# r9y9/gantts

Measured on NVIDIA H100. Metric: gan_step_frames_per_sec, higher is better.
Workload: dtype f32 (GEMMs: bf16x3 split on wgmma, fp32 accumulate)

## Files before the change

### gantts_b200/csrc/gan_step.cu

```cuda
#include <nvtx3/nvToolsExt.h>

#include "common.cuh"

namespace gantts {

struct NvtxRange {
  explicit NvtxRange(const char* name) { nvtxRangePushA(name); }
  ~NvtxRange() { nvtxRangePop(); }
};

enum ScalarSlot {
  S_REAL = 0,
  S_FAKE = 3,
  S_ADV = 6,
  S_MGE = 9,
  S_MSE = 11,
  S_DSUMSQ = 13,
  S_GSUMSQ = 14,
  S_INV_T = 15,
  S_ADV_SCALE = 16,
  S_MGE_SCALE = 17,
  S_MSE_SCALE = 18,
  S_COUNT = 32
};

__global__ void gather_cols_list_kernel(const float* __restrict__ in, int64_t in_rs, float* __restrict__ out,
                                        int64_t out_rs, ColList cols, int64_t rows) {
  __shared__ int sc[GANTTS_MAX_COLS];
  for (int i = threadIdx.x; i < cols.n; i += blockDim.x) sc[i] = cols.c[i];
  __syncthreads();
  const int lane = threadIdx.x & 31;
  const int64_t warp = ((int64_t)blockIdx.x * blockDim.x + threadIdx.x) >> 5;
  const int64_t nwarps = ((int64_t)gridDim.x * blockDim.x) >> 5;
  for (int64_t r = warp; r < rows; r += nwarps)
    for (int j = lane; j < cols.n; j += 32) out[r * out_rs + j] = in[r * in_rs + sc[j]];
}

__global__ void gather_planes_kernel(const float* __restrict__ a, int64_t a_rs, ColList ca, int64_t rows_a,
                                     const float* __restrict__ b, int64_t b_rs, ColList cb, int64_t rows_b,
                                     __nv_bfloat16* __restrict__ hi, __nv_bfloat16* __restrict__ lo, int64_t pitch) {
  pdl_entry();
  __shared__ int sa[GANTTS_MAX_COLS], sb[GANTTS_MAX_COLS];
  for (int i = threadIdx.x; i < ca.n; i += blockDim.x) sa[i] = ca.c[i];
  for (int i = threadIdx.x; i < cb.n; i += blockDim.x) sb[i] = cb.c[i];
  __syncthreads();
  const int lane = threadIdx.x & 31;
  const int64_t warp = ((int64_t)blockIdx.x * blockDim.x + threadIdx.x) >> 5;
  const int64_t nwarps = ((int64_t)gridDim.x * blockDim.x) >> 5;
  for (int64_t r = warp; r < rows_a + rows_b; r += nwarps) {
    const bool first = r < rows_a;
    const float* src = first ? a + r * a_rs : b + (r - rows_a) * b_rs;
    const int* sc = first ? sa : sb;
    const int n = first ? ca.n : cb.n;
    uint32_t* hr = reinterpret_cast<uint32_t*>(hi + r * pitch);
    uint32_t* lr = reinterpret_cast<uint32_t*>(lo + r * pitch);
    for (int c = 2 * lane; c < n; c += 64) {
      const float v0 = src[sc[c]], v1 = (c + 1 < n) ? src[sc[c + 1]] : 0.f;
      const uint32_t hp = pack_bf16x2(v0, v1);
      hr[c >> 1] = hp;
      lr[c >> 1] = pack_bf16x2(v0 - __uint_as_float(hp << 16), v1 - __uint_as_float(hp & 0xffff0000u));
    }
  }
}

__global__ void scatter_cols_list_add_kernel(const float* __restrict__ go, int64_t go_rs, float* __restrict__ gi,
                                             int64_t gi_rs, ColList cols, int64_t rows) {
  __shared__ int sc[GANTTS_MAX_COLS];
  for (int i = threadIdx.x; i < cols.n; i += blockDim.x) sc[i] = cols.c[i];
  __syncthreads();
  const int lane = threadIdx.x & 31;
  const int64_t warp = ((int64_t)blockIdx.x * blockDim.x + threadIdx.x) >> 5;
  const int64_t nwarps = ((int64_t)gridDim.x * blockDim.x) >> 5;
  for (int64_t r = warp; r < rows; r += nwarps)
    for (int j = lane; j < cols.n; j += 32) gi[r * gi_rs + sc[j]] += go[r * go_rs + j];
}

__global__ void set_scales_kernel(float* scal, float inv_frames, float adv_w, float mge_w, float mse_w,
                                  int zero_norms, const int64_t* __restrict__ lengths, int B, int T) {
  pdl_entry();
  if (threadIdx.x == 0) {
    if (zero_norms) scal[S_DSUMSQ] = scal[S_GSUMSQ] = 0.f;
    if (!(inv_frames > 0.f)) {
      int64_t n = 0;
      for (int b = 0; b < B; ++b) {
        const int64_t l = lengths[b];
        n += l < 0 ? 0 : (l > T ? T : l);
      }
      inv_frames = n > 0 ? 1.f / (float)n : 0.f;
    }
    scal[S_INV_T] = inv_frames;
    scal[S_ADV_SCALE] = adv_w * inv_frames;
    scal[S_MGE_SCALE] = mge_w * inv_frames;
    scal[S_MSE_SCALE] = mse_w * inv_frames;
  }
}

__global__ void __launch_bounds__(RED_THREADS)
spoof_count_kernel(const float* __restrict__ Dv, const int64_t* __restrict__ lengths, int B, int T, float* __restrict__ count) {
  pdl_entry();
  __shared__ float sm[32];
  float v[1] = {0.f};
  const int64_t rows = (int64_t)B * T;
  for (int64_t r = threadIdx.x; r < rows; r += RED_THREADS) {
    const int64_t t = r % T;
    if (t < lengths[r / T] && Dv[r] > 0.5f) v[0] += 1.f;
  }
  block_sum<1>(v, sm);
  if (threadIdx.x == 0) count[0] = v[0];
}

enum RedSlot { R_REAL = 0, R_FAKE = 1, R_ADV = 2, R_MGE = 3, R_MSE = 4, R_COUNT = 5 };

struct RedCounts {
  int n[R_COUNT];
};

__global__ void __launch_bounds__(RED_THREADS)
finalize_losses_kernel(const float* scal, float* losses, const RedWs* red, RedCounts cnt, float adv_w, float mge_w,
                       float mse_w, int has_d) {
  pdl_entry();
  __shared__ float sm[RED_NV * 32];
  __shared__ float tot[R_COUNT][RED_NV];
  for (int sl = 0; sl < R_COUNT; ++sl) {
    float v[RED_NV] = {0.f, 0.f, 0.f, 0.f};
    for (int i = threadIdx.x; i < cnt.n[sl]; i += RED_THREADS) {
#pragma unroll
      for (int k = 0; k < RED_NV; ++k) v[k] += red[sl].partial[i][k];
    }
    block_sum<RED_NV>(v, sm);
    if (threadIdx.x == 0) {
#pragma unroll
      for (int k = 0; k < RED_NV; ++k) tot[sl][k] = v[k];
    }
    __syncthreads();
  }
  if (threadIdx.x != 0) return;
  const float invT = scal[S_INV_T];
  const float real = has_d ? tot[R_REAL][0] * invT : 0.f, fake = has_d ? tot[R_FAKE][0] * invT : 0.f;
  const float adv = (has_d && adv_w > 0.f) ? tot[R_ADV][0] * invT : 0.f;
  const float mge = tot[R_MGE][0] * invT, mse = tot[R_MSE][0] * invT;
  losses[0] = real + fake;
  losses[1] = fake;
  losses[2] = real;
  losses[3] = mse;
  losses[4] = mge;
  losses[5] = adv;
  losses[6] = (mse_w * mse + mge_w * mge) + adv_w * adv;
  losses[7] = has_d ? tot[R_REAL][1] : 0.f;
  losses[8] = has_d ? tot[R_FAKE][1] : 0.f;
  losses[9] = tot[R_MGE][1];
  losses[10] = has_d ? sqrtf(scal[S_DSUMSQ]) : 0.f;
  losses[11] = sqrtf(scal[S_GSUMSQ]);
}

static inline int blocks_1d(int64_t work, int per_block) {
  int64_t b = (work + per_block - 1) / per_block;
  if (b < 1) b = 1;
  if (b > 132 * 8) b = 132 * 8;
  return (int)b;
}

static_assert(GANTTS_MAX_STEP_TENSORS == OPT_MAX_TENSORS, "one model's tensor table is one TensorList of the clip kernels");
static_assert(2 + 2 * GANTTS_MAX_LAYERS <= GANTTS_MAX_STEP_TENSORS && 2 * GANTTS_MAX_SRU_LAYERS + 2 <= GANTTS_MAX_STEP_TENSORS &&
                  2 + 8 * GANTTS_MAX_LSTM_LAYERS + 2 <= GANTTS_MAX_STEP_TENSORS,
              "every generator the step accepts fits one tensor table");

struct Bound {
  float* p;
  float* g;
};
enum { WEIGHT = 0, BIAS = 1 };
enum { W_IH = 0, W_HH = 1, B_IH = 2, B_HH = 3 };

struct ParamList {
  int n;
  float* p[GANTTS_MAX_STEP_TENSORS];
  float* g[GANTTS_MAX_STEP_TENSORS];
  float* s[GANTTS_MAX_STEP_TENSORS];
  float* s2[GANTTS_MAX_STEP_TENSORS];
  int64_t sizes[GANTTS_MAX_STEP_TENSORS];
  int64_t total;
  Bound gate[2];
  Bound sru[GANTTS_MAX_SRU_LAYERS][2];
  Bound lstm[GANTTS_MAX_LSTM_LAYERS][2][4];
  float* gW[GANTTS_MAX_LAYERS];
  float* gb[GANTTS_MAX_LAYERS];
};

static inline size_t al256(size_t v) { return (v + 255) / 256 * 256; }

struct Arena {
  char* cur;
  char* take(size_t bytes) {
    char* p = cur;
    cur += al256(bytes);
    return p;
  }
  float* f32(size_t n) { return reinterpret_cast<float*>(take(n * sizeof(float))); }
};

struct HighwayWs {
  float* tx;
  float* gx;
  char* w;
  char* dz;
  float* partial;
};

struct SruWs {
  char* in[GANTTS_MAX_SRU_LAYERS];
  float* u[GANTTS_MAX_SRU_LAYERS];
  float* c[GANTTS_MAX_SRU_LAYERS];
  float* h[GANTTS_MAX_SRU_LAYERS];
  char* w[GANTTS_MAX_SRU_LAYERS];
  float* partial[GANTTS_MAX_SRU_LAYERS];
  char* du;
  float* dx;
  float* dxp;
  float* bpart;
};

struct LstmWs {
  char* in[GANTTS_MAX_LSTM_LAYERS];
  char* w[GANTTS_MAX_LSTM_LAYERS];
  float* bias[GANTTS_MAX_LSTM_LAYERS];
  float* h[GANTTS_MAX_LSTM_LAYERS];
  float* gates[GANTTS_MAX_LSTM_LAYERS];
  float* cells[GANTTS_MAX_LSTM_LAYERS];
  float* xproj;
  float* out;
  float* dh;
  char* dg;
  char* hp;
  float* part[2][2];
  unsigned int* bar;
  int64_t* lengths;
};

struct StepLayout {
  float* scal;
  float* mask;
  float* d_in;
  float* d_out;
  float* g_dout;
  float* g_din;
  float* g_static;
  float* g_yhat;
  float* g_grads;
  float* d_grads;
  char* g_tape;
  size_t g_tape_bytes;
  char* d_tape;
  size_t d_tape_bytes;
  char* mlp_ws;
  size_t mlp_ws_bytes;
  RedWs* red;
  float* opt_partial;
  HighwayWs hw;
  SruWs sru;
  LstmWs lstm;
  LstmWs d_lstm;
  size_t total;
};

static inline int sru_ncols(const gantts_sru_stack_t& s) { return s.hidden * (s.bidirectional ? 2 : 1); }
static inline int sru_nin(const gantts_sru_stack_t& s, int l) { return l == 0 ? s.in_dim : sru_ncols(s); }
static inline int sru_k(const gantts_sru_stack_t& s, int l) { return sru_nin(s, l) != sru_ncols(s) ? 4 : 3; }
static inline int lstm_ndir(const gantts_lstm_stack_t& s) { return s.bidirectional ? 2 : 1; }
static inline int lstm_nin(const gantts_lstm_stack_t& s, int l) { return l == 0 ? s.in_dim : lstm_ndir(s) * s.hidden; }

static inline int gen_in_width(const gantts_gan_step_t* c) {
  return c->sru.num_layers > 0 ? c->sru.in_dim : (c->lstm.num_layers > 0 ? c->lstm.in_dim : c->g.dims[0]);
}

static inline int d_in_width(const gantts_gan_step_t* c) {
  return c->d_lstm.num_layers > 0 ? c->d_lstm.in_dim : c->d.dims[0];
}

static Bound take_tensor(const gantts_step_tensors_t& t, int64_t size, float* flat, ParamList* pl) {
  const int i = pl->n++;
  const Bound b{t.param[i], flat ? flat + pl->total : nullptr};
  pl->p[i] = b.p;
  pl->g[i] = b.g;
  pl->s[i] = t.state[i];
  pl->s2[i] = t.state2[i];
  pl->sizes[i] = size;
  pl->total += size;
  return b;
}

static void bind_mlp(const gantts_step_tensors_t& t, gantts_mlp_t* m, float* flat, ParamList* pl) {
  for (int l = 0; l < m->num_layers; ++l) {
    const Bound w = take_tensor(t, (int64_t)m->dims[l + 1] * m->dims[l], flat, pl);
    const Bound b = take_tensor(t, m->dims[l + 1], flat, pl);
    m->W[l] = w.p;
    m->b[l] = b.p;
    pl->gW[l] = w.g;
    pl->gb[l] = b.g;
  }
}

static void bind_lstm(const gantts_step_tensors_t& t, const gantts_lstm_stack_t& ls, float* flat, ParamList* pl) {
  const int64_t G4 = 4 * (int64_t)ls.hidden;
  for (int l = 0; l < ls.num_layers; ++l)
    for (int d = 0; d < lstm_ndir(ls); ++d) {
      const int64_t sizes[4] = {G4 * lstm_nin(ls, l), G4 * ls.hidden, G4, G4};
      for (int i = 0; i < 4; ++i) pl->lstm[l][d][i] = take_tensor(t, sizes[i], flat, pl);
    }
}

static void g_param_list(const gantts_gan_step_t* c, gantts_mlp_t* g, float* flat, ParamList* pl) {
  pl->n = 0;
  pl->total = 0;
  const gantts_step_tensors_t& t = c->g_tensors;
  const gantts_sru_stack_t& s = c->sru;
  for (int l = 0; l < s.num_layers; ++l) {
    pl->sru[l][WEIGHT] = take_tensor(t, (int64_t)sru_nin(s, l) * sru_ncols(s) * sru_k(s, l), flat, pl);
    pl->sru[l][BIAS] = take_tensor(t, 2 * (int64_t)sru_ncols(s), flat, pl);
  }
  const int64_t S = c->highway.static_dim;
  if (S > 0) {
    pl->gate[WEIGHT] = take_tensor(t, S * S, flat, pl);
    pl->gate[BIAS] = take_tensor(t, S, flat, pl);
  }
  bind_lstm(t, c->lstm, flat, pl);
  bind_mlp(t, g, flat, pl);
}

static void d_param_list(const gantts_gan_step_t* c, gantts_mlp_t* d, float* flat, ParamList* pl) {
  pl->n = 0;
  pl->total = 0;
  bind_lstm(c->d_tensors, c->d_lstm, flat, pl);
  bind_mlp(c->d_tensors, d, flat, pl);
}

static int64_t d_param_count(const gantts_gan_step_t* c) {
  ParamList pl;
  gantts_mlp_t d = c->d;
  d_param_list(c, &d, nullptr, &pl);
  return pl.total;
}

static int64_t g_param_count(const gantts_gan_step_t* c) {
  ParamList pl;
  gantts_mlp_t g = c->g;
  g_param_list(c, &g, nullptr, &pl);
  return pl.total;
}

struct OptSpec {
  int kind;
  float beta1, beta2, eps;
  int64_t step;
};
static OptSpec g_opt_spec(const gantts_gan_step_t* c) { return {c->optimizer, c->beta1, c->beta2, c->eps, c->opt_step}; }
static OptSpec d_opt_spec(const gantts_gan_step_t* c) {
  const gantts_optimizer_t& o = c->d_opt;
  return o.own ? OptSpec{o.optimizer, o.beta1, o.beta2, o.eps, o.opt_step} : g_opt_spec(c);
}

static int clip_opt_model(const gantts_gan_step_t* c, const OptSpec& o, const ParamList& pl, float* partial, float* sumsq_out,
                          float lr, float wd, cudaStream_t st) {
  TensorList tl;
  const bool adam = o.kind == GANTTS_OPT_ADAM;
  int rc = fill(tl, pl.p, pl.g, pl.s, adam ? pl.s2 : nullptr, pl.sizes, 0, pl.n);
  if (rc) return rc;
  const int nb = blocks_for(tl.off[tl.n], OPT_MAX_BLOCKS);
  GANTTS_PDL_LAUNCH((sumsq_partial_kernel), nb, OPT_THREADS, 0, st, tl, partial);
  GANTTS_LAUNCH_CHECK("sumsq_partial_kernel");
  if (adam) {
    GANTTS_CHECK_ARG(o.step >= 1, "gan_step: Adam needs opt_step >= 1 (the number of the step being taken)");
    const AdamScales a = adam_scales(lr, o.beta1, o.beta2, o.step);
    GANTTS_PDL_LAUNCH((clip_adam_partials_kernel), nb, OPT_THREADS, 0, st, tl, partial, nb, sumsq_out, c->max_norm, o.beta1, o.beta2,
                      wd, o.eps, a.step_size, a.inv_sqrt_bc2);
    GANTTS_LAUNCH_CHECK("clip_adam_partials_kernel");
  } else {
    GANTTS_PDL_LAUNCH((clip_adagrad_partials_kernel), nb, OPT_THREADS, 0, st, tl, partial, nb, sumsq_out, c->max_norm, lr, wd, o.eps);
    GANTTS_LAUNCH_CHECK("clip_adagrad_partials_kernel");
  }
  return GANTTS_OK;
}

static int check_table(const gantts_step_tensors_t& t, int want, int kind, const char* model) {
  GANTTS_CHECK_ARG(t.n == want, "gan_step: the %s table has %d tensors, its shapes give %d", model, t.n, want);
  for (int i = 0; i < t.n; ++i) {
    GANTTS_CHECK_ARG(t.param[i], "gan_step: null %s tensor %d", model, i);
    GANTTS_CHECK_ARG(t.state[i], "gan_step: null %s optimiser state of tensor %d", model, i);
    if (kind == GANTTS_OPT_ADAM)
      GANTTS_CHECK_ARG(t.state2[i], "gan_step: Adam needs exp_avg_sq for %s tensor %d", model, i);
  }
  return GANTTS_OK;
}

static int check_step(const gantts_gan_step_t* c) {
  GANTTS_CHECK_ARG(c, "gan_step: null config");
  GANTTS_CHECK_ARG(c->B >= 1 && c->T >= 1, "gan_step: bad batch shape");
  GANTTS_CHECK_ARG(c->optimizer == GANTTS_OPT_ADAGRAD || c->optimizer == GANTTS_OPT_ADAM, "gan_step: unknown optimizer %d", c->optimizer);
  if (c->optimizer == GANTTS_OPT_ADAM)
    GANTTS_CHECK_ARG(c->beta1 >= 0.f && c->beta1 < 1.f && c->beta2 >= 0.f && c->beta2 < 1.f, "gan_step: Adam betas out of range");
  const gantts_optimizer_t& dopt = c->d_opt;
  GANTTS_CHECK_ARG(dopt.own == 0 || dopt.own == 1, "gan_step: d_opt.own must be 0 (follow the step's optimiser) or 1 (got %d)",
                   dopt.own);
  if (dopt.own) {
    GANTTS_CHECK_ARG(dopt.optimizer == GANTTS_OPT_ADAGRAD || dopt.optimizer == GANTTS_OPT_ADAM,
                     "gan_step: unknown discriminator optimizer %d (d_opt.optimizer)", dopt.optimizer);
    if (dopt.optimizer == GANTTS_OPT_ADAM) {
      GANTTS_CHECK_ARG(dopt.beta1 >= 0.f && dopt.beta1 < 1.f && dopt.beta2 >= 0.f && dopt.beta2 < 1.f,
                       "gan_step: discriminator Adam betas out of range (d_opt.beta1 %g, d_opt.beta2 %g: each in [0, 1))",
                       (double)dopt.beta1, (double)dopt.beta2);
      GANTTS_CHECK_ARG(dopt.opt_step >= 1,
                       "gan_step: discriminator Adam needs d_opt.opt_step >= 1 (the number of the step being taken; got %lld)",
                       (long long)dopt.opt_step);
    }
  }
  GANTTS_CHECK_ARG(c->g.num_layers >= 1 && c->g.num_layers <= GANTTS_MAX_LAYERS, "gan_step: bad generator");
  GANTTS_CHECK_ARG(c->n_static >= 1 && c->n_static <= GANTTS_MAX_COLS, "gan_step: bad n_static");
  GANTTS_CHECK_ARG(c->n_static_cols == c->n_static, "gan_step: static column list must have n_static entries");
  const gantts_lstm_stack_t& ls = c->lstm;
  GANTTS_CHECK_ARG(ls.num_layers >= 0 && ls.num_layers <= GANTTS_MAX_LSTM_LAYERS,
                   "gan_step: LSTM layer count %d not in [0, %d] (train larger stacks with GanTrainer)", ls.num_layers,
                   GANTTS_MAX_LSTM_LAYERS);
  if (ls.num_layers > 0) {
    GANTTS_CHECK_ARG(c->highway.static_dim > 0,
                     "gan_step: an LSTM stack runs only with the highway gate (In2OutRNNHighwayNet); LSTMRNN and GRURNN "
                     "train with GanTrainer");
    GANTTS_CHECK_ARG(c->sru.num_layers == 0, "gan_step: the LSTM stack and the SRU stack are mutually exclusive");
    GANTTS_CHECK_ARG(ls.in_dim >= 1 && (ls.bidirectional == 0 || ls.bidirectional == 1),
                     "gan_step: bad LSTM shape (in_dim %d, bidirectional %d)", ls.in_dim, ls.bidirectional);
    GANTTS_CHECK_ARG(ls.hidden >= 4 && ls.hidden % 4 == 0, "gan_step: LSTM hidden size %d is not a positive multiple of 4",
                     ls.hidden);
    GANTTS_CHECK_ARG(c->B <= LSTM_MAX_B, "gan_step: an LSTM stack runs at most LSTM_MAX_B = %d sequences (B = %d)",
                     LSTM_MAX_B, c->B);
    GANTTS_CHECK_ARG(ls.dropout >= 0.f && ls.dropout < 1.f, "gan_step: LSTM dropout out of [0, 1)");
    const int nh = lstm_ndir(ls) * ls.hidden;
    GANTTS_CHECK_ARG(c->g.num_layers == 1 && c->g.dims[0] == nh,
                     "gan_step: with an LSTM stack g is hidden2out alone: 1 layer of input width %d (got %d layer(s), "
                     "input width %d)", nh, c->g.num_layers, c->g.dims[0]);
    GANTTS_CHECK_ARG(ls.in_dim == c->g.dims[1],
                     "gan_step: LSTM in_dim %d != hidden2out output width %d (the model returns its input as y_hat)",
                     ls.in_dim, c->g.dims[1]);
    if (int rc = lstm_check_trainable(ls.hidden, lstm_ndir(ls))) return rc;
  }
  const gantts_sru_stack_t& s = c->sru;
  GANTTS_CHECK_ARG(s.num_layers >= 0 && s.num_layers <= GANTTS_MAX_SRU_LAYERS, "gan_step: SRU layer count %d not in [0, %d]",
                   s.num_layers, GANTTS_MAX_SRU_LAYERS);
  if (s.num_layers > 0) {
    GANTTS_CHECK_ARG(c->highway.static_dim == 0, "gan_step: the SRU stack and the highway gate are mutually exclusive");
    GANTTS_CHECK_ARG(s.in_dim >= 1 && s.hidden >= 1 && (s.bidirectional == 0 || s.bidirectional == 1),
                     "gan_step: bad SRU shape (in_dim %d, hidden %d, bidirectional %d)", s.in_dim, s.hidden, s.bidirectional);
    GANTTS_CHECK_ARG(s.act >= 0 && s.act <= 2, "gan_step: SRU activation %d not in 0..2", s.act);
    GANTTS_CHECK_ARG(s.dropout >= 0.f && s.dropout < 1.f && s.rnn_dropout >= 0.f && s.rnn_dropout < 1.f,
                     "gan_step: SRU dropout / rnn_dropout out of [0, 1)");
    const int nc = sru_ncols(s);
    GANTTS_CHECK_ARG(c->g.num_layers == 1 && c->g.dims[0] == nc,
                     "gan_step: with an SRU stack g is hidden2out alone: 1 layer of input width %d (got %d layer(s), input "
                     "width %d)", nc, c->g.num_layers, c->g.dims[0]);
  }
  const gantts_lstm_stack_t& dl = c->d_lstm;
  GANTTS_CHECK_ARG(dl.num_layers >= 0 && dl.num_layers <= GANTTS_MAX_LSTM_LAYERS,
                   "gan_step: discriminator LSTM layer count %d not in [0, %d] (train larger stacks with GanTrainer)",
                   dl.num_layers, GANTTS_MAX_LSTM_LAYERS);
  if (c->w_d > 0.f) {
    GANTTS_CHECK_ARG(c->d.num_layers >= 1 && c->d.num_layers <= GANTTS_MAX_LAYERS, "gan_step: bad discriminator");
    if (dl.num_layers > 0) {
      GANTTS_CHECK_ARG(dl.bidirectional == 0 || dl.bidirectional == 1, "gan_step: bad discriminator LSTM bidirectional %d",
                       dl.bidirectional);
      GANTTS_CHECK_ARG(dl.hidden >= 4 && dl.hidden % 4 == 0,
                       "gan_step: discriminator LSTM hidden size %d is not a positive multiple of 4 (train it with GanTrainer)",
                       dl.hidden);
      GANTTS_CHECK_ARG(2 * c->B <= LSTM_MAX_B,
                       "gan_step: a recurrent discriminator runs the stacked [real | fake] batch of 2B sequences, at most "
                       "LSTM_MAX_B = %d, so B <= %d (B = %d); GanTrainer runs real and fake separately", LSTM_MAX_B,
                       LSTM_MAX_B / 2, c->B);
      GANTTS_CHECK_ARG(dl.dropout >= 0.f && dl.dropout < 1.f, "gan_step: discriminator LSTM dropout out of [0, 1)");
      const int nh = lstm_ndir(dl) * dl.hidden;
      GANTTS_CHECK_ARG(c->d.num_layers == 1 && c->d.dims[0] == nh,
                       "gan_step: with a discriminator LSTM stack d is hidden2out alone: 1 layer of input width %d (got %d "
                       "layer(s), input width %d)", nh, c->d.num_layers, c->d.dims[0]);
      if (int rc = lstm_check_trainable(dl.hidden, lstm_ndir(dl))) return rc;
    }
    const int cond_w = c->d_conditioned ? gen_in_width(c) : 0;
    GANTTS_CHECK_ARG(c->n_adv >= 1 && c->n_adv <= GANTTS_MAX_COLS && d_in_width(c) == cond_w + c->n_adv,
                     "gan_step: discriminator input width %d != %d conditioning + %d adversarial columns",
                     d_in_width(c), cond_w, c->n_adv);
    GANTTS_CHECK_ARG(c->d.dims[c->d.num_layers] == 1 && c->d.last_act == GANTTS_ACT_SIGMOID,
                     "gan_step: discriminator must end in a single sigmoid output");
  }
  GANTTS_CHECK_ARG(c->g.last_act == GANTTS_ACT_NONE, "gan_step: generator must have a linear output");
  GANTTS_CHECK_ARG(c->mlpg_table, "gan_step: null MLPG table");
  const gantts_highway_t& h = c->highway;
  GANTTS_CHECK_ARG(h.static_dim >= 0, "gan_step: negative highway static_dim");
  if (h.static_dim > 0) {
    const int S = h.static_dim, nw = c->windows.n, Lg = c->g.num_layers;
    const gantts_streams_t& st = c->streams;
    GANTTS_CHECK_ARG(st.n == 1 && st.dyn[0] && st.in_start[0] == 0 && st.out_start[0] == 0 && st.sd[0] == S,
                     "gan_step: a highway generator needs exactly one dynamic stream with in_start = out_start = 0 and "
                     "sd = static_dim = %d (got %d stream(s), first sd %d)", S, st.n, st.sd[0]);
    GANTTS_CHECK_ARG(c->n_static == S, "gan_step: highway static_dim %d != n_static %d", S, c->n_static);
    GANTTS_CHECK_ARG(gen_in_width(c) >= S, "gan_step: highway generator input width %d < static_dim %d", gen_in_width(c),
                     S);
    GANTTS_CHECK_ARG(c->g.dims[Lg] == nw * S, "gan_step: highway generator output width %d != %d windows x static_dim %d",
                     c->g.dims[Lg], nw, S);
  }
  ParamList pl;
  gantts_mlp_t g = c->g;
  g_param_list(c, &g, nullptr, &pl);
  int rc = check_table(c->g_tensors, pl.n, c->optimizer, "generator");
  if (rc) return rc;
  if (h.static_dim > 0)
    GANTTS_CHECK_ARG((reinterpret_cast<uintptr_t>(pl.gate[BIAS].p) & 15) == 0,
                     "gan_step: highway gate bias must be 16-byte aligned");
  if (!(c->w_d > 0.f)) return GANTTS_OK;
  gantts_mlp_t d = c->d;
  d_param_list(c, &d, nullptr, &pl);
  return check_table(c->d_tensors, pl.n, d_opt_spec(c).kind, "discriminator");
}

static void layout_lstm(const gantts_lstm_stack_t& ls, int64_t M, int out_cols, int64_t seqs, Arena& a, LstmWs* w,
                        bool bwd = true) {
  const int nl = ls.num_layers, H = nl > 0 ? ls.hidden : 0, nd = lstm_ndir(ls), n4 = nd * 4 * H;
  const bool on = nl > 0, on_bwd = on && bwd;
  size_t part_ih = 0, part_hh = 0;
  for (int l = 0; l < nl; ++l) {
    const int ni = lstm_nin(ls, l);
    w->in[l] = a.take(2 * plane_bytes(M, ni));
    w->w[l] = a.take(2 * plane_bytes(n4, ni) + 2 * plane_bytes(ni, n4));
    w->bias[l] = a.f32((size_t)n4);
    w->h[l] = a.f32((size_t)M * nd * H);
    w->gates[l] = a.f32((size_t)M * n4);
    w->cells[l] = a.f32((size_t)M * nd * H);
    const size_t pi = mn_partial_bytes_upto(M, 4 * H, ni), ph = mn_partial_bytes_upto(M, 4 * H, H);
    part_ih = pi > part_ih ? pi : part_ih;
    part_hh = ph > part_hh ? ph : part_hh;
  }
  w->xproj = a.f32((size_t)M * n4);
  w->out = a.f32(on ? (size_t)M * out_cols : 0);
  w->dh = a.f32(bwd ? (size_t)M * nd * H : 0);
  w->dg = a.take(on_bwd ? 2 * plane_bytes(M, n4) : 0);
  w->hp = a.take(on_bwd ? 2 * plane_bytes(M, H) : 0);
  for (int d = 0; d < 2; ++d) {
    w->part[d][0] = reinterpret_cast<float*>(a.take(bwd && d < nd ? part_ih : 0));
    w->part[d][1] = reinterpret_cast<float*>(a.take(bwd && d < nd ? part_hh : 0));
  }
  w->bar = reinterpret_cast<unsigned int*>(a.take(on ? 256 : 0));
  w->lengths = reinterpret_cast<int64_t*>(a.take(on ? (size_t)seqs * sizeof(int64_t) : 0));
}

struct LstmStack {
  const gantts_lstm_stack_t* s;
  const LstmWs* w;
  const Bound (*p)[2][4];
  int which;
  uint64_t mask_seed(uint64_t seed, int l) const {
    return which == 0 ? gantts_lstm_mask_seed(seed, l) : gantts_d_lstm_mask_seed(seed, which, l);
  }
};

static Planes lstm_in_planes(const LstmStack& k, int l, int64_t M) {
  char* cur = k.w->in[l];
  return carve_planes(cur, M, lstm_nin(*k.s, l));
}
static void lstm_w_planes(const LstmStack& k, int l, Planes* w, Planes* wt) {
  const int ni = lstm_nin(*k.s, l), n4 = lstm_ndir(*k.s) * 4 * k.s->hidden;
  char* cur = k.w->w[l];
  *w = carve_planes(cur, n4, ni);
  *wt = carve_planes(cur, ni, n4);
}

static LstmStack g_lstm(const gantts_gan_step_t* c, const StepLayout& L, const ParamList& pg) {
  return LstmStack{&c->lstm, &L.lstm, pg.lstm, 0};
}

static void layout_highway(const gantts_gan_step_t* c, int64_t M, Arena& a, HighwayWs* w) {
  const int S = c->highway.static_dim;
  const bool on = S > 0;
  w->tx = a.f32(on ? (size_t)M * S : 0);
  w->gx = a.f32(on ? (size_t)M * S : 0);
  w->w = a.take(on ? 2 * plane_bytes(S, S) : 0);
  w->dz = a.take(on ? 2 * plane_bytes(M, S) : 0);
  w->partial = reinterpret_cast<float*>(a.take(on ? mn_partial_bytes_upto(M, S, S) : 0));
}

static int gate_input_planes(const gantts_gan_step_t* c, const gantts_mlp_t& g, const StepLayout& L, int64_t M,
                             Planes* xs) {
  if (c->lstm.num_layers > 0) {
    *xs = lstm_in_planes(LstmStack{&c->lstm, &L.lstm, nullptr, 0}, 0, M);
  } else {
    int rc = mlp_tape_input_planes(&g, M, L.g_tape, L.g_tape_bytes, xs);
    if (rc) return rc;
  }
  xs->cols = c->highway.static_dim;
  return GANTTS_OK;
}

static int highway_gate_fwd(const gantts_gan_step_t* c, const gantts_mlp_t& g, const ParamList& pg, const StepLayout& L,
                            int64_t M, cudaStream_t st) {
  const int S = c->highway.static_dim;
  Planes xs;
  int rc = gate_input_planes(c, g, L, M, &xs);
  if (rc) return rc;
  char* cur = L.hw.w;
  const Planes w = carve_planes(cur, S, S);
  if ((rc = launch_split(pg.gate[WEIGHT].p, S, S, S, w, 0, st))) return rc;
  EpiArgs e;
  e.epi = EPI_F32;
  e.C = L.hw.tx;
  e.ldc = S;
  e.bias = pg.gate[BIAS].p;
  e.act = GANTTS_ACT_SIGMOID;
  return launch_gemm_kk(xs, w, e, st);
}

static int highway_gate_bwd(const gantts_gan_step_t* c, const gantts_mlp_t& g, const ParamList& pg, const StepLayout& L,
                            int64_t M, cudaStream_t st) {
  const int S = c->highway.static_dim;
  Planes xs;
  int rc = gate_input_planes(c, g, L, M, &xs);
  if (rc) return rc;
  char* cur = L.hw.dz;
  const Planes dz = carve_planes(cur, M, S);
  ReduceList rl;
  if ((rc = launch_gemm_mn(dz, xs, pg.gate[WEIGHT].g, pg.gate[BIAS].g, 0, L.hw.partial, st, &rl))) return rc;
  return flush_reduce(rl, 0, st);
}

static void layout_sru(const gantts_gan_step_t* c, int64_t M, Arena& a, SruWs* w) {
  const gantts_sru_stack_t& s = c->sru;
  const int nl = s.num_layers, nc = nl > 0 ? sru_ncols(s) : 0;
  int maxku = 0;
  for (int l = 0; l < nl; ++l) {
    const int ni = sru_nin(s, l), ku = nc * sru_k(s, l);
    maxku = ku > maxku ? ku : maxku;
    w->in[l] = a.take(2 * plane_bytes(M, ni));
    w->u[l] = a.f32((size_t)M * ku);
    w->c[l] = a.f32((size_t)M * nc);
    if (l < nl - 1) w->h[l] = a.f32((size_t)M * nc);
    w->w[l] = a.take(2 * plane_bytes(ni, ku) + 2 * plane_bytes(ku, ni));
    w->partial[l] = reinterpret_cast<float*>(a.take(mn_partial_bytes_upto(M, ni, ku)));
  }
  w->du = a.take(nl > 0 ? 2 * plane_bytes(M, maxku) : 0);
  w->dx = a.f32((size_t)M * nc);
  w->dxp = a.f32((size_t)M * nc);
  w->bpart = a.f32((size_t)c->B * 2 * nc);
}

static Planes sru_in_planes(const gantts_gan_step_t* c, const StepLayout& L, int l, int64_t M) {
  char* cur = L.sru.in[l];
  return carve_planes(cur, M, sru_nin(c->sru, l));
}
static void sru_w_planes(const gantts_gan_step_t* c, const StepLayout& L, int l, Planes* w, Planes* wt) {
  const int ni = sru_nin(c->sru, l), ku = sru_ncols(c->sru) * sru_k(c->sru, l);
  char* cur = L.sru.w[l];
  *w = carve_planes(cur, ni, ku);
  *wt = carve_planes(cur, ku, ni);
}

static int sru_stack_fwd(const gantts_gan_step_t* c, const gantts_mlp_t& g, const ParamList& pg, const StepLayout& L,
                         const float* x, int B, int T, uint64_t seed, bool train, cudaStream_t st) {
  const int64_t M = (int64_t)B * T;
  const gantts_sru_stack_t& s = c->sru;
  const int nl = s.num_layers, nc = sru_ncols(s);
  const float p_h = train ? s.dropout : 0.f, p_x = train ? s.rnn_dropout : 0.f;
  int rc;
  {
    WeightSplitList wl;
    wl.n = nl;
    wl.off[0] = 0;
    for (int l = 0; l < nl; ++l) {
      Planes w, wt;
      sru_w_planes(c, L, l, &w, &wt);
      wl.W[l] = pg.sru[l][WEIGHT].p;
      wl.N[l] = (int)w.rows;
      wl.K[l] = (int)w.cols;
      wl.hi[l] = w.hi;
      wl.lo[l] = w.lo;
      wl.pitch[l] = w.pitch;
      wl.thi[l] = wt.hi;
      wl.tlo[l] = wt.lo;
      wl.tpitch[l] = wt.pitch;
      wl.off[l + 1] = wl.off[l] + (int64_t)((w.rows + 31) / 32) * ((w.cols + 31) / 32);
    }
    int nb = (int)(wl.off[nl] < num_sms() * 8 ? wl.off[nl] : num_sms() * 8);
    GANTTS_PDL_LAUNCH((split_weights_kernel), nb < 1 ? 1 : nb, 256, 0, st, wl);
    GANTTS_LAUNCH_CHECK("split_weights_kernel(sru)");
  }
  const Planes in0 = sru_in_planes(c, L, 0, M);
  if (p_x > 0.f) {
    GANTTS_PDL_LAUNCH((sru_mask_split_kernel), blocks_1d(M * s.in_dim, 1024), 256, 0, st, x, (int64_t)s.in_dim, M, s.in_dim,
                      T, sru_mask(gantts_sru_mask_seed(seed, 0, 0), p_x), in0.hi, in0.lo, in0.pitch);
    GANTTS_LAUNCH_CHECK("sru_mask_split_kernel");
  } else if ((rc = launch_split(x, s.in_dim, M, s.in_dim, in0, 0, st))) {
    return rc;
  }
  Planes top;
  if ((rc = mlp_tape_input_planes(&g, M, L.g_tape, L.g_tape_bytes, &top))) return rc;
  for (int l = 0; l < nl; ++l) {
    const int k = sru_k(s, l);
    const bool last = l == nl - 1;
    Planes w, wt;
    sru_w_planes(c, L, l, &w, &wt);
    EpiArgs e;
    e.epi = EPI_F32;
    e.C = L.sru.u[l];
    e.ldc = (int64_t)nc * k;
    if ((rc = launch_gemm_kk(sru_in_planes(c, L, l, M), wt, e, st))) return rc;
    const Planes out = last ? top : sru_in_planes(c, L, l + 1, M);
    SruStepFwd p{};
    p.u = L.sru.u[l];
    p.xh = k == 3 ? (l == 0 ? x : L.sru.h[l - 1]) : nullptr;
    p.xh_rs = l == 0 ? s.in_dim : nc;
    p.bias = pg.sru[l][BIAS].p;
    p.c = L.sru.c[l];
    p.h = L.sru.h[l];
    p.hi = out.hi;
    p.lo = out.lo;
    p.pitch = out.pitch;
    p.mh = sru_mask(gantts_sru_mask_seed(seed, l, 1), last ? 0.f : p_h);
    p.mx = sru_mask(gantts_sru_mask_seed(seed, l + 1, 0), last ? 0.f : p_x);
    p.B = B;
    p.T = T;
    p.d = s.hidden;
    p.bidir = s.bidirectional;
    p.act = s.act;
    if ((rc = launch_sru_step_fwd(p, k, st))) return rc;
  }
  return GANTTS_OK;
}

static int sru_stack_bwd(const gantts_gan_step_t* c, const StepLayout& L, const ParamList& pg, const float* x, int B, int T,
                         uint64_t seed, cudaStream_t st) {
  const int64_t M = (int64_t)B * T;
  const gantts_sru_stack_t& s = c->sru;
  const int nl = s.num_layers, nc = sru_ncols(s);
  int rc;
  ReduceList rl;
  for (int l = nl - 1; l >= 0; --l) {
    const int k = sru_k(s, l);
    const bool top = l == nl - 1;
    char* cur = L.sru.du;
    const Planes du = carve_planes(cur, M, (int64_t)nc * k);
    SruStepBwd p{};
    p.u = L.sru.u[l];
    p.xh = k == 3 ? (l == 0 ? x : L.sru.h[l - 1]) : nullptr;
    p.xh_rs = l == 0 ? s.in_dim : nc;
    p.bias = pg.sru[l][BIAS].p;
    p.c = L.sru.c[l];
    p.dx = L.sru.dx;
    p.dxp_in = top ? nullptr : L.sru.dxp;
    p.mxu = sru_mask(gantts_sru_mask_seed(seed, l + 1, 0), top ? 0.f : s.rnn_dropout);
    p.mh = sru_mask(gantts_sru_mask_seed(seed, l, 1), top ? 0.f : s.dropout);
    p.du_hi = du.hi;
    p.du_lo = du.lo;
    p.du_pitch = du.pitch;
    p.dxp_out = (k == 3 && l > 0) ? L.sru.dxp : nullptr;
    p.dbias_part = L.sru.bpart;
    p.B = B;
    p.T = T;
    p.d = s.hidden;
    p.bidir = s.bidirectional;
    p.act = s.act;
    if ((rc = launch_sru_step_bwd(p, k, st))) return rc;
    GANTTS_PDL_LAUNCH((sru_bias_reduce_kernel), (2 * nc + 255) / 256, 256, 0, st, L.sru.bpart, B, 2 * nc, pg.sru[l][BIAS].g);
    GANTTS_LAUNCH_CHECK("sru_bias_reduce_kernel");
    if ((rc = launch_gemm_mn(sru_in_planes(c, L, l, M), du, pg.sru[l][WEIGHT].g, nullptr, 0, L.sru.partial[l], st, &rl))) return rc;
    if (l > 0) {
      Planes w, wt;
      sru_w_planes(c, L, l, &w, &wt);
      EpiArgs e;
      e.epi = EPI_F32;
      e.C = L.sru.dx;
      e.ldc = nc;
      if ((rc = launch_gemm_kk(du, w, e, st))) return rc;
    }
  }
  return flush_reduce(rl, 0, st);
}

static LstmParams lstm_layer_params(const LstmStack& k, int l, const int64_t* lengths, int B, int T) {
  const gantts_lstm_stack_t& s = *k.s;
  LstmParams p{};
  p.W_hh = k.p[l][0][W_HH].p;
  if (s.bidirectional)
    p.W_hh_dir = ((int64_t)reinterpret_cast<uintptr_t>(k.p[l][1][W_HH].p) - (int64_t)reinterpret_cast<uintptr_t>(k.p[l][0][W_HH].p)) /
                 (int64_t)sizeof(float);
  p.lengths = lengths;
  p.h_out = k.w->h[l];
  p.gates = k.w->gates[l];
  p.cells = k.w->cells[l];
  p.bar = k.w->bar;
  p.B = B;
  p.T = T;
  p.H = s.hidden;
  p.ndir = lstm_ndir(s);
  return p;
}

static int lstm_stack_fwd(const LstmStack& k, const float* x, int64_t x_rs, const Planes& top, const int64_t* lengths,
                          int B, int T, uint64_t seed, bool train, cudaStream_t st) {
  const int64_t M = (int64_t)B * T;
  const gantts_lstm_stack_t& s = *k.s;
  const int nl = s.num_layers, H = s.hidden, nd = lstm_ndir(s), G4 = 4 * H, nh = nd * H;
  const float p_drop = train ? s.dropout : 0.f;
  int rc;
  {
    WeightSplitList wl;
    LstmBiasList bl;
    wl.n = bl.n = nl * nd;
    wl.off[0] = 0;
    bl.len = G4;
    for (int l = 0; l < nl; ++l) {
      Planes w, wt;
      lstm_w_planes(k, l, &w, &wt);
      for (int d = 0; d < nd; ++d) {
        const int i = l * nd + d;
        wl.W[i] = k.p[l][d][W_IH].p;
        wl.N[i] = G4;
        wl.K[i] = lstm_nin(s, l);
        wl.hi[i] = w.hi + (int64_t)d * G4 * w.pitch;
        wl.lo[i] = w.lo + (int64_t)d * G4 * w.pitch;
        wl.pitch[i] = w.pitch;
        wl.thi[i] = wt.hi + (int64_t)d * G4;
        wl.tlo[i] = wt.lo + (int64_t)d * G4;
        wl.tpitch[i] = wt.pitch;
        wl.off[i + 1] = wl.off[i] + (int64_t)((G4 + 31) / 32) * ((wl.K[i] + 31) / 32);
        bl.a[i] = k.p[l][d][B_IH].p;
        bl.b[i] = k.p[l][d][B_HH].p;
        bl.out[i] = k.w->bias[l] + (int64_t)d * G4;
      }
    }
    const int nb = (int)(wl.off[wl.n] < num_sms() * 8 ? wl.off[wl.n] : num_sms() * 8);
    GANTTS_PDL_LAUNCH((split_weights_kernel), nb < 1 ? 1 : nb, 256, 0, st, wl);
    GANTTS_LAUNCH_CHECK("split_weights_kernel(lstm)");
    GANTTS_PDL_LAUNCH((lstm_bias_sum_kernel), (bl.n * G4 + 255) / 256, 256, 0, st, bl);
    GANTTS_LAUNCH_CHECK("lstm_bias_sum_kernel");
  }
  if (x && (rc = launch_split(x, x_rs, M, s.in_dim, lstm_in_planes(k, 0, M), 0, st))) return rc;
  for (int l = 0; l < nl; ++l) {
    const bool last = l == nl - 1;
    Planes w, wt;
    lstm_w_planes(k, l, &w, &wt);
    EpiArgs e;
    e.epi = EPI_F32;
    e.C = k.w->xproj;
    e.ldc = (int64_t)nd * G4;
    e.bias = k.w->bias[l];
    if ((rc = launch_gemm_kk(lstm_in_planes(k, l, M), w, e, st))) return rc;
    LstmParams p = lstm_layer_params(k, l, lengths, B, T);
    p.xproj = k.w->xproj;
    if ((rc = lstm_run(false, p, st))) return rc;
    const Planes out = last ? top : lstm_in_planes(k, l + 1, M);
    const float pl = last ? 0.f : p_drop;
    GANTTS_PDL_LAUNCH((lstm_planes_kernel), blocks_1d(M * nh, 1024), 256, 0, st, k.w->h[l], M, nh,
                      k.mask_seed(seed, l), pl > 0.f ? (uint32_t)(pl * 65536.f + 0.5f) : 0u,
                      pl > 0.f ? 1.f / (1.f - pl) : 1.f, out.hi, out.lo, out.pitch);
    GANTTS_LAUNCH_CHECK("lstm_planes_kernel");
  }
  return GANTTS_OK;
}

struct LstmInGrad {
  int64_t row0;
  int col0, cols;
  float* C;
  int64_t ldc;
  int accumulate;
};

static int lstm_stack_bwd(const LstmStack& k, const int64_t* lengths, int B, int T, uint64_t seed, bool param_grads,
                          const LstmInGrad* din, cudaStream_t st) {
  const int64_t M = (int64_t)B * T;
  const gantts_lstm_stack_t& s = *k.s;
  const int nl = s.num_layers, H = s.hidden, nd = lstm_ndir(s), G4 = 4 * H, nh = nd * H;
  int rc;
  char* cur = k.w->dg;
  const Planes dg = carve_planes(cur, M, (int64_t)nd * G4);
  cur = k.w->hp;
  const Planes hp = carve_planes(cur, M, H);
  ReduceList rl;
  for (int l = nl - 1; l >= 0; --l) {
    LstmParams p = lstm_layer_params(k, l, lengths, B, T);
    p.dh_out = k.w->dh;
    p.dxproj = k.w->xproj;
    if ((rc = lstm_run(true, p, st))) return rc;
    if ((rc = launch_split(k.w->xproj, (int64_t)nd * G4, M, nd * G4, dg, 0, st))) return rc;
    const Planes in = lstm_in_planes(k, l, M);
    for (int d = 0; d < nd && param_grads; ++d) {
      Planes dgd = dg;
      dgd.hi += (int64_t)d * G4;
      dgd.lo += (int64_t)d * G4;
      dgd.cols = G4;
      if ((rc = launch_gemm_mn(dgd, in, k.p[l][d][W_IH].g, k.p[l][d][B_IH].g, 0, k.w->part[d][0], st, &rl))) return rc;
      GANTTS_PDL_LAUNCH((lstm_hprev_planes_kernel), blocks_1d(M * H, 1024), 256, 0, st, k.w->h[l], lengths, B, T, H, nd,
                        d, hp.hi, hp.lo, hp.pitch);
      GANTTS_LAUNCH_CHECK("lstm_hprev_planes_kernel");
      if ((rc = launch_gemm_mn(dgd, hp, k.p[l][d][W_HH].g, nullptr, 0, k.w->part[d][1], st, &rl))) return rc;
    }
    if (l > 0) {
      Planes w, wt;
      lstm_w_planes(k, l, &w, &wt);
      EpiArgs e;
      e.epi = EPI_F32;
      e.C = k.w->dh;
      e.ldc = nh;
      if (s.dropout > 0.f) {
        e.act = GANTTS_ACT_LEAKY_DROPOUT;
        e.slope = 1.f;
        e.p = s.dropout;
        e.seed = k.mask_seed(seed, l - 1);
      }
      if ((rc = launch_gemm_kk(dg, wt, e, st))) return rc;
    } else if (din) {
      Planes w, wt;
      lstm_w_planes(k, 0, &w, &wt);
      Planes a = dg;
      a.hi += din->row0 * dg.pitch;
      a.lo += din->row0 * dg.pitch;
      a.rows = M - din->row0;
      wt.hi += (int64_t)din->col0 * wt.pitch;
      wt.lo += (int64_t)din->col0 * wt.pitch;
      wt.rows = din->cols;
      EpiArgs e;
      e.epi = EPI_F32;
      e.C = din->C;
      e.ldc = din->ldc;
      e.accumulate = din->accumulate;
      if ((rc = launch_gemm_kk(a, wt, e, st))) return rc;
    }
    if (!param_grads) continue;
    if ((rc = flush_reduce(rl, 0, st))) return rc;
    for (int d = 0; d < nd; ++d)
      GANTTS_CUDA(cudaMemcpyAsync(k.p[l][d][B_HH].g, k.p[l][d][B_IH].g, (size_t)G4 * sizeof(float), cudaMemcpyDeviceToDevice, st));
  }
  return GANTTS_OK;
}

static void layout(const gantts_gan_step_t* c, char* base, StepLayout* L) {
  const int64_t M = (int64_t)c->B * c->T;
  const int dD = d_in_width(c);
  *L = StepLayout{};
  Arena a{base};
  L->scal = a.f32(S_COUNT);
  L->mask = a.f32((size_t)M);
  L->d_in = a.f32((size_t)2 * M * dD);
  L->d_out = a.f32((size_t)2 * M);
  L->g_dout = a.f32((size_t)2 * M);
  L->g_din = a.f32((size_t)2 * M * dD);
  L->g_static = a.f32((size_t)M * c->n_static);
  L->g_yhat = a.f32((size_t)M * c->g.dims[c->g.num_layers]);
  L->g_grads = a.f32(g_param_count(c));
  L->d_grads = a.f32(d_param_count(c));
  L->g_tape_bytes = gantts_mlp_tape_bytes(&c->g, M);
  L->g_tape = a.take(L->g_tape_bytes);
  L->d_tape_bytes = gantts_mlp_tape_bytes(&c->d, 2 * M);
  L->d_tape = a.take(L->d_tape_bytes);
  const size_t gb = mlp_workspace_bytes(&c->g, M, true), db = mlp_workspace_bytes(&c->d, 2 * M, true);
  L->mlp_ws_bytes = gb > db ? gb : db;
  L->mlp_ws = a.take(L->mlp_ws_bytes);
  L->red = reinterpret_cast<RedWs*>(a.take(R_COUNT * sizeof(RedWs)));
  L->opt_partial = a.f32(OPT_MAX_BLOCKS);
  layout_highway(c, M, a, &L->hw);
  layout_sru(c, M, a, &L->sru);
  layout_lstm(c->lstm, M, c->g.dims[c->g.num_layers], 0, a, &L->lstm);
  layout_lstm(c->d_lstm, 2 * M, 0, 2 * (int64_t)c->B, a, &L->d_lstm);
  L->total = (size_t)(a.cur - base) + 256;
}

struct Step {
  const gantts_gan_step_t* c;
  StepLayout L;
  int B, T;
  const float* table;
  gantts_mlp_t g, d;
  ParamList pg, pd;
  const float *x, *y;
  const int64_t* lengths;
  float *y_hat, *y_hat_static;
  int64_t M;
  int d_in, d_out, dD, nS;
  int cond_w, nA;
  bool has_d, has_adv;
  bool train;
  bool adv_window;
  HighwayArgs hwa;
  ColList static_cols, adv_cols, real_cols;
  uint64_t seed;
  void* stream;
  cudaStream_t st;
  const HighwayArgs* hw() const { return c->highway.static_dim > 0 ? &hwa : nullptr; }
  bool d_rnn() const { return c->d_lstm.num_layers > 0; }
  LstmStack d_lstm(int which) const { return LstmStack{&c->d_lstm, &L.d_lstm, pd.lstm, which}; }
};

static int step_prologue(const Step& s, float inv_frames, bool zero_norms) {
  const gantts_gan_step_t* c = s.c;
  int rc = gantts_sequence_mask(s.lengths, s.L.mask, s.B, s.T, s.stream);
  if (rc) return rc;
  GANTTS_PDL_LAUNCH((set_scales_kernel), 1, 32, 0, s.st, s.L.scal, inv_frames, s.has_adv ? c->adv_w : 0.f, c->mge_w, c->mse_w,
                    zero_norms ? 1 : 0, s.lengths, s.B, s.T);
  GANTTS_LAUNCH_CHECK("set_scales_kernel");
  return GANTTS_OK;
}

static int step_finalize(const Step& s, float* losses_dev) {
  const gantts_gan_step_t* c = s.c;
  RedCounts cnt{};
  if (s.has_d) cnt.n[R_REAL] = cnt.n[R_FAKE] = bce_blocks(s.M);
  if (s.has_adv) cnt.n[R_ADV] = bce_blocks(s.M);
  cnt.n[R_MGE] = sse_blocks(s.M, s.nS);
  cnt.n[R_MSE] = sse_blocks(s.M, s.d_out);
  GANTTS_PDL_LAUNCH((finalize_losses_kernel), 1, RED_THREADS, 0, s.st, s.L.scal, losses_dev, s.L.red, cnt,
                    s.has_adv ? c->adv_w : 0.f, c->mge_w, c->mse_w, s.has_d ? 1 : 0);
  GANTTS_LAUNCH_CHECK("finalize_losses_kernel");
  return GANTTS_OK;
}

static int generator_fwd(Step& s, bool train) {
  const gantts_gan_step_t* c = s.c;
  const StepLayout& L = s.L;
  const int64_t M = s.M;
  const float* gen_out = s.y_hat;
  int rc;
  if (c->lstm.num_layers > 0) {
    Planes top;
    if ((rc = mlp_tape_input_planes(&s.g, M, L.g_tape, L.g_tape_bytes, &top))) return rc;
    if ((rc = lstm_stack_fwd(g_lstm(c, L, s.pg), s.x, s.d_in, top, s.lengths, s.B, s.T, s.seed, train, s.st))) return rc;
    if ((rc = mlp_fwd_impl(&s.g, nullptr, 0, M, L.lstm.out, s.d_out, L.g_tape, L.g_tape_bytes, s.st, true))) return rc;
    GANTTS_CUDA(cudaMemcpyAsync(s.y_hat, s.x, (size_t)M * s.d_in * sizeof(float), cudaMemcpyDeviceToDevice, s.st));
    gen_out = L.lstm.out;
  } else if (c->sru.num_layers > 0) {
    if ((rc = sru_stack_fwd(c, s.g, s.pg, L, s.x, s.B, s.T, s.seed, train, s.st))) return rc;
    if ((rc = mlp_fwd_impl(&s.g, nullptr, 0, M, s.y_hat, s.d_out, L.g_tape, L.g_tape_bytes, s.st, true))) return rc;
  } else if ((rc = gantts_mlp_fwd(&s.g, s.x, s.d_in, M, s.y_hat, s.d_out, L.g_tape, L.g_tape_bytes, s.st))) {
    return rc;
  }
  if (c->highway.static_dim > 0 && (rc = highway_gate_fwd(c, s.g, s.pg, L, M, s.st))) return rc;
  return mlpg_fwd_impl(gen_out, (int64_t)s.T * s.d_out, s.d_out, s.y_hat_static, (int64_t)s.T * s.nS, s.nS, s.table,
                       &c->streams, &c->windows, s.B, s.T, s.stream, s.hw());
}

static int generator_bwd(Step& s) {
  const gantts_gan_step_t* c = s.c;
  const StepLayout& L = s.L;
  const int64_t M = s.M;
  const int d_out = s.d_out, nS = s.nS;
  const bool sru = c->sru.num_layers > 0, lstm = c->lstm.num_layers > 0;
  const bool mse_grad = c->mse_w != 0.f && !lstm;
  int rc;
  if ((rc = launch_sse(s.y_hat, d_out, s.y, d_out, L.mask, M, d_out, L.scal + S_MSE_SCALE, mse_grad ? L.g_yhat : nullptr,
                       d_out, &L.red[R_MSE], s.st)))
    return rc;
  bool direct = false;
  if (!mse_grad) {
    Planes gp;
    if ((rc = mlp_bwd_gy_planes(&s.g, M, L.mlp_ws, L.mlp_ws_bytes, &gp))) return rc;
    rc = mlpg_bwd_planes(L.g_static, (int64_t)s.T * nS, nS, gp.hi, gp.lo, gp.pitch, s.table, &c->streams,
                         &c->windows, s.B, s.T, s.stream, s.hw());
    if (rc == GANTTS_OK) direct = true;
    else if (rc != GANTTS_E_UNSUPPORTED) return rc;
  }
  if (!direct &&
      (rc = mlpg_bwd_impl(L.g_static, (int64_t)s.T * nS, nS, L.g_yhat, (int64_t)s.T * d_out, d_out, s.table,
                          &c->streams, &c->windows, s.B, s.T, mse_grad ? 1 : 0, s.stream, s.hw())))
    return rc;
  if (c->highway.static_dim > 0 && (rc = highway_gate_bwd(c, s.g, s.pg, L, M, s.st))) return rc;
  float* gx = sru ? L.sru.dx : (lstm ? L.lstm.dh : nullptr);
  const int gx_rs = sru ? sru_ncols(c->sru) : (lstm ? lstm_ndir(c->lstm) * c->lstm.hidden : 0);
  if ((rc = mlp_bwd_impl(&s.g, direct ? nullptr : L.g_yhat, d_out, nullptr, 0, M, L.g_tape, L.g_tape_bytes, gx, gx_rs, 0,
                         s.pg.gW, s.pg.gb, 0, L.mlp_ws, L.mlp_ws_bytes, s.stream, -1, direct)))
    return rc;
  if (sru) return sru_stack_bwd(c, L, s.pg, s.x, s.B, s.T, s.seed, s.st);
  if (lstm) return lstm_stack_bwd(g_lstm(c, L, s.pg), s.lengths, s.B, s.T, s.seed, true, nullptr, s.st);
  return GANTTS_OK;
}

static int discriminator_stack_fwd(Step& s, bool stacked, const float* x, const Planes& top) {
  const int64_t* lengths = s.lengths;
  if (stacked) {
    lengths = s.L.d_lstm.lengths;
    for (int half = 0; half < 2; ++half)
      GANTTS_CUDA(cudaMemcpyAsync(s.L.d_lstm.lengths + half * s.B, s.lengths, (size_t)s.B * sizeof(int64_t),
                                  cudaMemcpyDeviceToDevice, s.st));
  }
  return lstm_stack_fwd(s.d_lstm(stacked ? 1 : 2), x, s.dD, top, lengths, stacked ? 2 * s.B : s.B, s.T, s.seed, s.train,
                        s.st);
}

static int discriminator_fwd(Step& s, bool stacked) {
  const StepLayout& L = s.L;
  const int64_t M = s.M, rows = stacked ? 2 * M : M;
  int rc;
  Planes tape_in;
  if ((rc = mlp_tape_input_planes(&s.d, rows, L.d_tape, L.d_tape_bytes, &tape_in))) return rc;
  const Planes din = s.d_rnn() ? lstm_in_planes(s.d_lstm(stacked ? 1 : 2), 0, rows) : tape_in;
  if (!s.cond_w) {
    if (stacked) {
      GANTTS_PDL_LAUNCH((gather_planes_kernel), blocks_1d(2 * M * s.nA, 1024), 256, 0, s.st, s.y, s.d_out, s.real_cols, M,
                        s.y_hat_static, s.nS, s.adv_cols, M, din.hi, din.lo, din.pitch);
      GANTTS_LAUNCH_CHECK("gather_planes_kernel(real|fake)");
    } else {
      ColList none;
      none.n = 0;
      GANTTS_PDL_LAUNCH((gather_planes_kernel), blocks_1d(M * s.nA, 1024), 256, 0, s.st, s.y_hat_static, s.nS, s.adv_cols, M,
                        nullptr, 0, none, 0, din.hi, din.lo, din.pitch);
      GANTTS_LAUNCH_CHECK("gather_planes_kernel(adv)");
    }
    if (s.d_rnn() && (rc = discriminator_stack_fwd(s, stacked, nullptr, tape_in))) return rc;
    return mlp_fwd_impl(&s.d, nullptr, 0, rows, L.d_out, 1, L.d_tape, L.d_tape_bytes, s.stream, true);
  }
  const int dD = s.dD;
  if (stacked) {
    gather_cols_list_kernel<<<blocks_1d(M * s.nA, 1024), 256, 0, s.st>>>(s.y, s.d_out, L.d_in + s.cond_w, dD, s.real_cols, M);
    GANTTS_LAUNCH_CHECK("gather_cols_list_kernel(real)");
    gather_cols_list_kernel<<<blocks_1d(M * s.nA, 1024), 256, 0, s.st>>>(s.y_hat_static, s.nS, L.d_in + M * dD + s.cond_w,
                                                                          dD, s.adv_cols, M);
    GANTTS_LAUNCH_CHECK("gather_cols_list_kernel(fake)");
    for (int64_t half = 0; half < 2; ++half)
      GANTTS_CUDA(cudaMemcpy2DAsync(L.d_in + half * M * dD, (size_t)dD * sizeof(float), s.x, (size_t)s.d_in * sizeof(float),
                                    (size_t)s.cond_w * sizeof(float), (size_t)M, cudaMemcpyDeviceToDevice, s.st));
  }
  if (s.d_rnn()) {
    if ((rc = discriminator_stack_fwd(s, stacked, L.d_in + (stacked ? 0 : M * dD), tape_in))) return rc;
    return mlp_fwd_impl(&s.d, nullptr, 0, rows, L.d_out, 1, L.d_tape, L.d_tape_bytes, s.stream, true);
  }
  return gantts_mlp_fwd(&s.d, L.d_in + (stacked ? 0 : M * dD), dD, rows, L.d_out, 1, L.d_tape, L.d_tape_bytes, s.stream);
}

static int discriminator_bwd(Step& s, bool stacked, bool input_grad = true) {
  const StepLayout& L = s.L;
  const int64_t M = s.M, skip = stacked ? M : 0;
  float* const* gW = stacked ? s.pd.gW : nullptr;
  float* const* gb = stacked ? s.pd.gb : nullptr;
  float* gx = !input_grad ? nullptr : (s.adv_window ? L.g_static + s.adv_cols.c[0] - skip * (int64_t)s.nS : L.g_din);
  int rc;
  if (s.d_rnn()) {
    const LstmStack k = s.d_lstm(stacked ? 1 : 2);
    const int nh = lstm_ndir(s.c->d_lstm) * s.c->d_lstm.hidden;
    if ((rc = mlp_bwd_impl(&s.d, L.g_dout, 1, L.d_out, 1, skip + M, L.d_tape, L.d_tape_bytes, k.w->dh, nh, 0, gW, gb, 0,
                           L.mlp_ws, L.mlp_ws_bytes, s.stream, 0)))
      return rc;
    LstmInGrad din{};
    if (input_grad) {
      const int64_t rs = s.adv_window ? s.nS : s.dD;
      din = LstmInGrad{skip, s.cond_w, s.nA, (s.adv_window ? gx : gx + s.cond_w) + skip * rs, rs, s.adv_window ? 1 : 0};
    }
    if ((rc = lstm_stack_bwd(k, stacked ? L.d_lstm.lengths : s.lengths, stacked ? 2 * s.B : s.B, s.T, s.seed, stacked,
                             input_grad ? &din : nullptr, s.st)))
      return rc;
  } else if ((rc = mlp_bwd_impl(&s.d, L.g_dout, 1, L.d_out, 1, skip + M, L.d_tape, L.d_tape_bytes, gx, s.adv_window ? s.nS : s.dD,
                                skip, gW, gb, 0, L.mlp_ws, L.mlp_ws_bytes, s.stream, s.adv_window ? 1 : -1))) {
    return rc;
  }
  if (s.adv_window || !input_grad) return GANTTS_OK;
  scatter_cols_list_add_kernel<<<blocks_1d(M * s.nA, 1024), 256, 0, s.st>>>(L.g_din + skip * s.dD + s.cond_w, s.dD,
                                                                             L.g_static, s.nS, s.adv_cols, M);
  GANTTS_LAUNCH_CHECK("scatter_cols_list_add_kernel");
  return GANTTS_OK;
}

}

using namespace gantts;

extern "C" uint64_t gantts_gan_step_seed(uint64_t seed, int which) { return seed * 4 + (uint64_t)which; }

extern "C" uint64_t gantts_sru_mask_seed(uint64_t seed, int layer, int which) {
  return gantts_mlp_layer_seed(gantts_gan_step_seed(seed, 3), 2 * layer + which);
}

extern "C" uint64_t gantts_lstm_mask_seed(uint64_t seed, int layer) {
  return gantts_mlp_layer_seed(gantts_gan_step_seed(seed, 3), 2 * GANTTS_MAX_SRU_LAYERS + layer);
}

extern "C" uint64_t gantts_d_lstm_mask_seed(uint64_t seed, int which, int layer) {
  return gantts_mlp_layer_seed(gantts_gan_step_seed(seed, 3),
                               2 * GANTTS_MAX_SRU_LAYERS + GANTTS_MAX_LSTM_LAYERS * which + layer);
}

extern "C" size_t gantts_gan_step_workspace_bytes(const gantts_gan_step_t* c) {
  if (check_step(c)) return 0;
  StepLayout L;
  layout(c, nullptr, &L);
  return L.total + 256;
}

extern "C" int gantts_gan_step_grad_buffer(const gantts_gan_step_t* c, void* workspace, int which, float** ptr,
                                           int64_t* count) {
  int rc = check_step(c);
  if (rc) return rc;
  GANTTS_CHECK_ARG(workspace && ptr && count, "gan_step_grad_buffer: null pointer");
  StepLayout L;
  layout(c, reinterpret_cast<char*>(al256(reinterpret_cast<uintptr_t>(workspace))), &L);
  *ptr = which == 0 ? L.g_grads : L.d_grads;
  *count = which == 0 ? g_param_count(c) : d_param_count(c);
  return GANTTS_OK;
}

extern "C" int gantts_gan_step(const gantts_gan_step_t* c, int phases, const float* x, const float* y,
                               const int64_t* lengths_dev, float inv_frames, uint64_t seed, float* y_hat,
                               float* y_hat_static, float* losses_dev, void* workspace, size_t workspace_bytes,
                               void* stream) {
  GANTTS_CHECK_ARG(c, "gan_step: null config");
  return gantts_gan_step_shaped(c, c->B, c->T, c->mlpg_table, phases, x, y, lengths_dev, inv_frames, seed, y_hat,
                                y_hat_static, losses_dev, workspace, workspace_bytes, stream);
}

extern "C" int gantts_gan_step_shaped(const gantts_gan_step_t* c, int B, int T, const float* mlpg_table, int phases,
                                      const float* x, const float* y, const int64_t* lengths_dev, float inv_frames,
                                      uint64_t seed, float* y_hat, float* y_hat_static, float* losses_dev, void* workspace,
                                      size_t workspace_bytes, void* stream) {
  int rc = check_step(c);
  if (rc) return rc;
  GANTTS_CHECK_ARG(B >= 1 && B <= c->B, "gan_step_shaped: batch size B = %d must be in [1, configured B = %d]", B, c->B);
  GANTTS_CHECK_ARG(T >= 1 && T <= c->T, "gan_step_shaped: padded length T = %d must be in [1, configured T = %d]", T, c->T);
  GANTTS_CHECK_ARG(mlpg_table, "gan_step_shaped: null MLPG table (it must be gantts_mlpg_table(windows, T) of the call's T)");
  const bool d_only = (phases & GANTTS_STEP_D_ONLY) != 0;
  if (d_only) {
    GANTTS_CHECK_ARG(!(phases & GANTTS_STEP_EVAL),
                     "gan_step: GANTTS_STEP_D_ONLY cannot be combined with GANTTS_STEP_EVAL (the test phase updates nothing)");
    GANTTS_CHECK_ARG(c->w_d > 0.f, "gan_step: GANTTS_STEP_D_ONLY trains the discriminator and needs w_d > 0 (got %g)",
                     (double)c->w_d);
  }
  GANTTS_CHECK_ARG(x && y && lengths_dev && y_hat && y_hat_static && losses_dev, "gan_step: null pointer");
  size_t need = gantts_gan_step_workspace_bytes(c);
  if (!workspace || workspace_bytes < need) {
    set_error("gan_step: workspace too small (%zu < %zu)", workspace_bytes, need);
    return GANTTS_E_WORKSPACE;
  }
  Step s;
  s.c = c;
  s.B = B;
  s.T = T;
  s.table = mlpg_table;
  s.stream = stream;
  s.st = as_stream(stream);
  layout(c, reinterpret_cast<char*>(al256(reinterpret_cast<uintptr_t>(workspace))), &s.L);
  const StepLayout& L = s.L;
  const int64_t M = s.M = (int64_t)B * T;
  s.x = x;
  s.y = y;
  s.lengths = lengths_dev;
  s.y_hat = y_hat;
  s.y_hat_static = y_hat_static;
  s.seed = seed;
  s.train = !(phases & GANTTS_STEP_EVAL);
  s.d_in = gen_in_width(c);
  s.d_out = c->g.dims[c->g.num_layers];
  s.dD = d_in_width(c);
  const int nS = s.nS = c->n_static;
  s.has_d = c->w_d > 0.f;
  s.has_adv = s.has_d && c->adv_w > 0.f && !d_only;
  s.cond_w = (s.has_d && c->d_conditioned) ? s.d_in : 0;
  s.nA = s.dD - s.cond_w;
  s.g = c->g;
  s.d = c->d;
  g_param_list(c, &s.g, L.g_grads, &s.pg);
  s.pd.n = 0;
  s.pd.total = 0;
  if (s.has_d) d_param_list(c, &s.d, L.d_grads, &s.pd);
  s.hwa = HighwayArgs{};
  if (c->highway.static_dim > 0) {
    char* cur = L.hw.dz;
    const Planes dz = carve_planes(cur, M, nS);
    s.hwa = HighwayArgs{x, s.d_in, L.hw.tx, L.hw.gx, dz.hi, dz.lo, dz.pitch, nS};
  }
  s.static_cols.n = c->n_static_cols;
  for (int i = 0; i < c->n_static_cols; ++i) s.static_cols.c[i] = c->static_cols[i];
  s.adv_cols.n = s.has_d ? c->n_adv : 0;
  for (int i = 0; i < s.adv_cols.n; ++i) s.adv_cols.c[i] = c->adv_cols[i];
  s.adv_window = s.has_d && !s.cond_w && s.adv_cols.n >= 1;
  for (int i = 1; i < s.adv_cols.n; ++i) s.adv_window = s.adv_window && s.adv_cols.c[i] == s.adv_cols.c[0] + i;
  s.real_cols.n = s.adv_cols.n;
  for (int i = 0; i < s.adv_cols.n; ++i) {
    GANTTS_CHECK_ARG(s.adv_cols.c[i] >= 0 && s.adv_cols.c[i] < c->n_static_cols, "gan_step: adversarial column out of range");
    s.real_cols.c[i] = s.static_cols.c[s.adv_cols.c[i]];
  }
  s.g.seed = gantts_gan_step_seed(seed, 0);
  const cudaStream_t st = s.st;

  if (phases & GANTTS_STEP_EVAL) {
    NvtxRange r_eval("gantts_gan_step/eval");
    GANTTS_CHECK_ARG(phases == GANTTS_STEP_EVAL, "gan_step: GANTTS_STEP_EVAL cannot be combined with training phases");
    s.g.dropout_p = 0.f;
    s.d.dropout_p = 0.f;
    if ((rc = step_prologue(s, inv_frames, true))) return rc;
    if ((rc = generator_fwd(s, false))) return rc;
    if (s.has_d) {
      if ((rc = discriminator_fwd(s, true))) return rc;
      if ((rc = launch_bce(L.d_out, L.mask, M, 2, 0, 1, L.scal + S_INV_T, nullptr, &L.red[R_REAL], &L.red[R_FAKE], st)))
        return rc;
      if (s.has_adv &&
          (rc = launch_bce(L.d_out + M, L.mask, M, 1, 0, 0, L.scal + S_INV_T, nullptr, &L.red[R_ADV], nullptr, st)))
        return rc;
    }
    if ((rc = launch_sse(y_hat_static, nS, y, s.d_out, L.mask, M, nS, L.scal + S_MGE_SCALE, nullptr, 0, &L.red[R_MGE], st,
                         &s.static_cols)))
      return rc;
    if ((rc = launch_sse(y_hat, s.d_out, y, s.d_out, L.mask, M, s.d_out, L.scal + S_MSE_SCALE, nullptr, 0, &L.red[R_MSE],
                         st)))
      return rc;
    return step_finalize(s, losses_dev);
  }

  if (phases & 1) {
    NvtxRange r1("gantts_gan_step/phase1: G fwd, MLPG, MGE, D fwd+bwd");
    if ((rc = step_prologue(s, inv_frames, d_only))) return rc;
    if ((rc = generator_fwd(s, true))) return rc;
    if ((rc = launch_sse(y_hat_static, nS, y, s.d_out, L.mask, M, nS, L.scal + S_MGE_SCALE, d_only ? nullptr : L.g_static, nS,
                         &L.red[R_MGE], st, &s.static_cols)))
      return rc;
    if (d_only && (rc = launch_sse(y_hat, s.d_out, y, s.d_out, L.mask, M, s.d_out, L.scal + S_MSE_SCALE, nullptr, 0,
                                   &L.red[R_MSE], st)))
      return rc;
    if (s.has_d) {
      s.d.seed = gantts_gan_step_seed(seed, 1);
      if ((rc = discriminator_fwd(s, true))) return rc;
      if ((rc = launch_bce(L.d_out, L.mask, M, 2, 0, 1, L.scal + S_INV_T, L.g_dout, &L.red[R_REAL], &L.red[R_FAKE], st)))
        return rc;
      if ((rc = discriminator_bwd(s, true, !d_only))) return rc;
    }
  }
  if (d_only) {
    if (phases & 2) {
      NvtxRange r2("gantts_gan_step/phase2 (D only): D step");
      if ((rc = clip_opt_model(c, d_opt_spec(c), s.pd, L.opt_partial, L.scal + S_DSUMSQ, c->lr_d, c->wd_d, st))) return rc;
    }
    if (phases & 4) {
      NvtxRange r4("gantts_gan_step/phase4 (D only): losses");
      return step_finalize(s, losses_dev);
    }
    return GANTTS_OK;
  }
  if (phases & 2) {
    NvtxRange r2("gantts_gan_step/phase2: D step, adv D fwd+bwd, MLPG bwd, G bwd");
    if (s.has_d && (rc = clip_opt_model(c, d_opt_spec(c), s.pd, L.opt_partial, L.scal + S_DSUMSQ, c->lr_d, c->wd_d, st)))
      return rc;
    if (s.has_adv) {
      s.d.seed = gantts_gan_step_seed(seed, 2);
      if ((rc = discriminator_fwd(s, false))) return rc;
      if ((rc = launch_bce(L.d_out, L.mask, M, 1, 0, 0, L.scal + S_ADV_SCALE, L.g_dout, &L.red[R_ADV], nullptr, st)))
        return rc;
      if ((rc = discriminator_bwd(s, false))) return rc;
    }
    if ((rc = generator_bwd(s))) return rc;
  }
  if (phases & 4) {
    NvtxRange r4("gantts_gan_step/phase4: G step, losses");
    if ((rc = clip_opt_model(c, g_opt_spec(c), s.pg, L.opt_partial, L.scal + S_GSUMSQ, c->lr_g, c->wd_g, st))) return rc;
    return step_finalize(s, losses_dev);
  }
  return GANTTS_OK;
}

static int check_spoof_d(const gantts_mlp_t* d, int64_t rows) {
  GANTTS_CHECK_ARG(d, "spoof_count: null reference discriminator");
  GANTTS_CHECK_ARG(d->num_layers >= 1 && d->num_layers <= GANTTS_MAX_LAYERS, "spoof_count: bad layer count %d", d->num_layers);
  GANTTS_CHECK_ARG(d->dims[d->num_layers] == 1 && d->last_act == GANTTS_ACT_SIGMOID,
                   "spoof_count: the reference discriminator must end in a single sigmoid output");
  GANTTS_CHECK_ARG(rows >= 1 && rows < (1 << 24),
                   "spoof_count: B * T = %lld frames, the float count is exact below 2^24", (long long)rows);
  return GANTTS_OK;
}

static int spoof_cols(const char* who, const int* adv_cols, int n_adv, int n_static, int d_width, ColList* cols) {
  GANTTS_CHECK_ARG(n_adv >= 1 && n_adv <= GANTTS_MAX_COLS && n_adv == d_width,
                   "%s: %d adversarial columns != reference discriminator input width %d (it gets no "
                   "linguistic conditioning, train.py:554-555)", who, n_adv, d_width);
  GANTTS_CHECK_ARG(n_static >= 1, "%s: bad n_static", who);
  cols->n = n_adv;
  for (int i = 0; i < n_adv; ++i) {
    GANTTS_CHECK_ARG(adv_cols[i] >= 0 && adv_cols[i] < n_static, "%s: adversarial column %d out of range", who,
                     adv_cols[i]);
    cols->c[i] = adv_cols[i];
  }
  return GANTTS_OK;
}

static int spoof_gather(const float* y_hat_static, int n_static, const ColList& cols, int64_t rows, const Planes& in,
                        cudaStream_t st) {
  ColList none;
  none.n = 0;
  GANTTS_PDL_LAUNCH((gather_planes_kernel), blocks_1d(rows * cols.n, 1024), 256, 0, st, y_hat_static, (int64_t)n_static, cols,
                    rows, nullptr, 0, none, 0, in.hi, in.lo, in.pitch);
  GANTTS_LAUNCH_CHECK("gather_planes_kernel(spoof)");
  return GANTTS_OK;
}

static int spoof_threshold(const float* dout, const int64_t* lengths_dev, int B, int T, float* count_dev, cudaStream_t st) {
  GANTTS_PDL_LAUNCH((spoof_count_kernel), 1, RED_THREADS, 0, st, dout, lengths_dev, B, T, count_dev);
  GANTTS_LAUNCH_CHECK("spoof_count_kernel");
  return GANTTS_OK;
}

extern "C" size_t gantts_spoof_count_workspace_bytes(const gantts_mlp_t* d, int64_t rows) {
  if (check_spoof_d(d, rows)) return 0;
  return al256(gantts_mlp_tape_bytes(d, rows)) + al256((size_t)rows * sizeof(float)) + 256;
}

extern "C" int gantts_spoof_count(const gantts_mlp_t* d, const float* y_hat_static, int n_static, const int* adv_cols,
                                  int n_adv, const int64_t* lengths_dev, int B, int T, float* count_dev, void* ws,
                                  size_t ws_bytes, void* stream) {
  GANTTS_CHECK_ARG(B >= 1 && T >= 1, "spoof_count: bad batch shape");
  const int64_t rows = (int64_t)B * T;
  int rc = check_spoof_d(d, rows);
  if (rc) return rc;
  GANTTS_CHECK_ARG(y_hat_static && adv_cols && lengths_dev && count_dev, "spoof_count: null pointer");
  ColList cols;
  if ((rc = spoof_cols("spoof_count", adv_cols, n_adv, n_static, d->dims[0], &cols))) return rc;
  const size_t need = gantts_spoof_count_workspace_bytes(d, rows);
  if (!ws || ws_bytes < need) {
    set_error("spoof_count: workspace too small (%zu < %zu)", ws_bytes, need);
    return GANTTS_E_WORKSPACE;
  }
  gantts_mlp_t m = *d;
  m.dropout_p = 0.f;
  char* base = reinterpret_cast<char*>(al256(reinterpret_cast<uintptr_t>(ws)));
  const size_t tape_bytes = gantts_mlp_tape_bytes(&m, rows);
  char* tape = base;
  float* dout = reinterpret_cast<float*>(base + al256(tape_bytes));
  const cudaStream_t st = as_stream(stream);
  Planes din;
  if ((rc = mlp_tape_input_planes(&m, rows, tape, tape_bytes, &din))) return rc;
  if ((rc = spoof_gather(y_hat_static, n_static, cols, rows, din, st))) return rc;
  if ((rc = mlp_fwd_impl(&m, nullptr, 0, rows, dout, 1, tape, tape_bytes, stream, true))) return rc;
  return spoof_threshold(dout, lengths_dev, B, T, count_dev, st);
}

struct SpoofLstmLayout {
  LstmWs lstm;
  char* tape;
  size_t tape_bytes;
  float* dout;
  size_t total;
};

static void layout_spoof_lstm(const gantts_lstm_stack_t& ls, const gantts_mlp_t& head, int64_t rows, char* base,
                              SpoofLstmLayout* L) {
  *L = SpoofLstmLayout{};
  Arena a{base};
  layout_lstm(ls, rows, 0, 0, a, &L->lstm, false);
  L->tape_bytes = gantts_mlp_tape_bytes(&head, rows);
  L->tape = a.take(L->tape_bytes);
  L->dout = a.f32((size_t)rows);
  L->total = (size_t)(a.cur - base);
}

static int check_spoof_lstm(const gantts_lstm_stack_t* ls, const gantts_mlp_t* head, int B, int T) {
  GANTTS_CHECK_ARG(ls && head, "spoof_count_lstm: null reference discriminator");
  GANTTS_CHECK_ARG(ls->num_layers >= 1 && ls->num_layers <= GANTTS_MAX_LSTM_LAYERS,
                   "spoof_count_lstm: LSTM layer count %d not in [1, %d] (count with GanTrainer)", ls->num_layers,
                   GANTTS_MAX_LSTM_LAYERS);
  GANTTS_CHECK_ARG(ls->hidden >= 4 && ls->hidden % 4 == 0,
                   "spoof_count_lstm: LSTM hidden size %d is not a positive multiple of 4", ls->hidden);
  GANTTS_CHECK_ARG(ls->bidirectional == 0 || ls->bidirectional == 1, "spoof_count_lstm: bad LSTM bidirectional %d",
                   ls->bidirectional);
  GANTTS_CHECK_ARG(ls->in_dim >= 1, "spoof_count_lstm: bad LSTM in_dim %d", ls->in_dim);
  GANTTS_CHECK_ARG(B >= 1 && T >= 1, "spoof_count_lstm: bad batch shape");
  GANTTS_CHECK_ARG(B <= LSTM_MAX_B, "spoof_count_lstm: an LSTM stack runs at most LSTM_MAX_B = %d sequences (B = %d)",
                   LSTM_MAX_B, B);
  GANTTS_CHECK_ARG((int64_t)B * T < (1 << 24), "spoof_count_lstm: B * T = %lld frames, the float count is exact below 2^24",
                   (long long)B * T);
  const int nh = lstm_ndir(*ls) * ls->hidden;
  GANTTS_CHECK_ARG(head->num_layers == 1 && head->dims[0] == nh && head->dims[1] == 1 && head->last_act == GANTTS_ACT_SIGMOID,
                   "spoof_count_lstm: the head must be hidden2out alone, 1 layer of %d -> 1 with a sigmoid (got %d "
                   "layer(s), input width %d)", nh, head->num_layers, head->dims[0]);
  return GANTTS_OK;
}

extern "C" size_t gantts_spoof_count_lstm_workspace_bytes(const gantts_lstm_stack_t* ls, const gantts_mlp_t* head, int B,
                                                          int T) {
  if (check_spoof_lstm(ls, head, B, T)) return 0;
  SpoofLstmLayout L;
  layout_spoof_lstm(*ls, *head, (int64_t)B * T, nullptr, &L);
  return L.total + 256;
}

extern "C" int gantts_spoof_count_lstm(const gantts_lstm_stack_t* ls, const float* const* lstm_tensors, int n_tensors,
                                       const gantts_mlp_t* head, const float* y_hat_static, int n_static,
                                       const int* adv_cols, int n_adv, const int64_t* lengths_dev, int B, int T,
                                       float* count_dev, void* ws, size_t ws_bytes, void* stream) {
  int rc = check_spoof_lstm(ls, head, B, T);
  if (rc) return rc;
  GANTTS_CHECK_ARG(lstm_tensors && y_hat_static && adv_cols && lengths_dev && count_dev && head->W[0] && head->b[0],
                   "spoof_count_lstm: null pointer");
  const int want = 4 * lstm_ndir(*ls) * ls->num_layers;
  GANTTS_CHECK_ARG(n_tensors == want,
                   "spoof_count_lstm: %d LSTM tensors, the stack has %d (W_ih, W_hh, b_ih, b_hh per layer and direction)",
                   n_tensors, want);
  for (int i = 0; i < n_tensors; ++i) GANTTS_CHECK_ARG(lstm_tensors[i], "spoof_count_lstm: null pointer (LSTM tensor %d)", i);
  ColList cols;
  if ((rc = spoof_cols("spoof_count_lstm", adv_cols, n_adv, n_static, ls->in_dim, &cols))) return rc;
  const size_t need = gantts_spoof_count_lstm_workspace_bytes(ls, head, B, T);
  if (!ws || ws_bytes < need) {
    set_error("spoof_count_lstm: workspace too small (%zu < %zu)", ws_bytes, need);
    return GANTTS_E_WORKSPACE;
  }
  const int64_t rows = (int64_t)B * T;
  SpoofLstmLayout L;
  layout_spoof_lstm(*ls, *head, rows, reinterpret_cast<char*>(al256(reinterpret_cast<uintptr_t>(ws))), &L);
  gantts_step_tensors_t t{};
  t.n = n_tensors;
  for (int i = 0; i < n_tensors; ++i) t.param[i] = const_cast<float*>(lstm_tensors[i]);
  ParamList pl;
  pl.n = 0;
  pl.total = 0;
  bind_lstm(t, *ls, nullptr, &pl);
  const LstmStack k{ls, &L.lstm, pl.lstm, 0};
  gantts_mlp_t m = *head;
  m.dropout_p = 0.f;
  const cudaStream_t st = as_stream(stream);
  if ((rc = spoof_gather(y_hat_static, n_static, cols, rows, lstm_in_planes(k, 0, rows), st))) return rc;
  Planes top;
  if ((rc = mlp_tape_input_planes(&m, rows, L.tape, L.tape_bytes, &top))) return rc;
  if ((rc = lstm_stack_fwd(k, nullptr, 0, top, lengths_dev, B, T, 0, false, st))) return rc;
  if ((rc = mlp_fwd_impl(&m, nullptr, 0, rows, L.dout, 1, L.tape, L.tape_bytes, stream, true))) return rc;
  return spoof_threshold(L.dout, lengths_dev, B, T, count_dev, st);
}
```

### gantts_b200/csrc/losses.cu

```cuda
#include "common.cuh"

namespace gantts {

constexpr int RED_THREADS = 256;
constexpr int RED_MAX_BLOCKS = 132 * 4;
constexpr int RED_NV = 4;

struct RedWs {
  float partial[RED_MAX_BLOCKS][RED_NV];
};

__global__ void sequence_mask_kernel(const int64_t* __restrict__ lengths, float* __restrict__ mask,
                                     int B, int T) {
  pdl_entry();
  int64_t i = (int64_t)blockIdx.x * blockDim.x + threadIdx.x;
  if (i >= (int64_t)B * T) return;
  int b = (int)(i / T), t = (int)(i - (int64_t)b * T);
  mask[i] = (int64_t)t < lengths[b] ? 1.f : 0.f;
}

struct ColList {
  int n;
  int c[GANTTS_MAX_COLS];
};

__global__ void __launch_bounds__(RED_THREADS)
sse_fwd_bwd_kernel(const float* __restrict__ a, int64_t a_rs, const float* __restrict__ b, int64_t b_rs,
                   const float* __restrict__ mask, int64_t rows, int D, const float* __restrict__ scale,
                   float* __restrict__ ga, int64_t ga_rs, RedWs* ws, ColList bmap) {
  pdl_entry();
  __shared__ float sm[RED_NV * 32];
  __shared__ int sc[GANTTS_MAX_COLS];
  for (int i = threadIdx.x; i < bmap.n; i += RED_THREADS) sc[i] = bmap.c[i];
  __syncthreads();
  const bool mapped = bmap.n > 0;
  float v[RED_NV] = {0.f, 0.f, 0.f, 0.f};
  const float s2 = ga ? 2.f * scale[0] : 0.f;
  const int lane = threadIdx.x & 31;
  const int64_t warp = ((int64_t)blockIdx.x * RED_THREADS + threadIdx.x) >> 5;
  const int64_t nwarps = ((int64_t)gridDim.x * RED_THREADS) >> 5;
  for (int64_t r = warp; r < rows; r += nwarps) {
    const float m = mask[r];
    const float* ar = a + r * a_rs;
    const float* br = b + r * b_rs;
#pragma unroll 4
    for (int d = lane; d < D; d += 32) {
      const float x = ar[d] * m - br[mapped ? sc[d] : d] * m;
      v[0] = fmaf(x, x, v[0]);
      if (ga) ga[r * ga_rs + d] = s2 * x * m;
    }
    if (lane == 0) v[1] += m;
  }
  block_sum<RED_NV>(v, sm);
  if (threadIdx.x == 0) {
#pragma unroll
    for (int k = 0; k < RED_NV; ++k) ws->partial[blockIdx.x][k] = v[k];
  }
}

__global__ void __launch_bounds__(RED_THREADS)
reduce_finish_kernel(const RedWs* ws, int nblocks, float* out, int nout) {
  __shared__ float sm[RED_NV * 32];
  float v[RED_NV] = {0.f, 0.f, 0.f, 0.f};
  for (int i = threadIdx.x; i < nblocks; i += RED_THREADS) {
#pragma unroll
    for (int k = 0; k < RED_NV; ++k) v[k] += ws->partial[i][k];
  }
  block_sum<RED_NV>(v, sm);
  if (threadIdx.x == 0)
    for (int k = 0; k < nout; ++k) out[k] = v[k];
}

__global__ void __launch_bounds__(RED_THREADS)
masked_sse_bwd_kernel(const float* __restrict__ a, int64_t a_rs, const float* __restrict__ b,
                      int64_t b_rs, const float* __restrict__ mask, int64_t rows, int D,
                      const float* __restrict__ scale, float* __restrict__ ga, int64_t ga_rs,
                      int accumulate) {
  const float s2 = 2.f * scale[0];
  const int lane = threadIdx.x & 31;
  const int64_t warp = ((int64_t)blockIdx.x * RED_THREADS + threadIdx.x) >> 5;
  const int64_t nwarps = ((int64_t)gridDim.x * RED_THREADS) >> 5;
  for (int64_t r = warp; r < rows; r += nwarps) {
    const float m = mask[r];
    const float* ar = a + r * a_rs;
    const float* br = b + r * b_rs;
    float* gr = ga + r * ga_rs;
#pragma unroll 4
    for (int d = lane; d < D; d += 32) {
      const float g = s2 * (ar[d] * m - br[d] * m) * m;
      gr[d] = accumulate ? gr[d] + g : g;
    }
  }
}

__global__ void __launch_bounds__(RED_THREADS)
bce_fwd_bwd_kernel(const float* __restrict__ Dv, const float* __restrict__ mask, int64_t M, int kind0, int kind1,
                   int nbh, const float* __restrict__ scale, float* __restrict__ gD, RedWs* ws0, RedWs* ws1) {
  pdl_entry();
  __shared__ float sm[RED_NV * 32];
  const int half = blockIdx.x >= nbh ? 1 : 0;
  const int kind = half ? kind1 : kind0;
  const int blk = blockIdx.x - half * nbh;
  const float* d = Dv + (int64_t)half * M;
  float* g = gD ? gD + (int64_t)half * M : nullptr;
  const float s = g ? scale[0] : 0.f;
  float v[RED_NV] = {0.f, 0.f, 0.f, 0.f};
  for (int64_t i = (int64_t)blk * RED_THREADS + threadIdx.x; i < M; i += (int64_t)nbh * RED_THREADS) {
    const float dv = d[i], m = mask[i];
    const float arg = kind == 0 ? (dv + 1e-20f) : (1.f - dv + 1e-20f);
    v[0] -= logf(arg) * m;
    const bool hit = kind == 0 ? (dv > 0.5f) : (dv < 0.5f);
    v[1] += hit ? m : 0.f;
    v[2] += m;
    if (g) g[i] = kind == 0 ? (-s * m / (dv + 1e-20f)) : (s * m / (1.f - dv + 1e-20f));
  }
  block_sum<RED_NV>(v, sm);
  if (threadIdx.x == 0) {
    RedWs* ws = half ? ws1 : ws0;
#pragma unroll
    for (int k = 0; k < RED_NV; ++k) ws->partial[blk][k] = v[k];
  }
}

__global__ void masked_bce_bwd_kernel(const float* __restrict__ Dv, const float* __restrict__ mask,
                                      int64_t rows, int kind, const float* __restrict__ scale,
                                      float* __restrict__ gD) {
  int64_t i = (int64_t)blockIdx.x * blockDim.x + threadIdx.x;
  if (i >= rows) return;
  float d = Dv[i], m = mask[i], s = scale[0];
  gD[i] = kind == 0 ? (-s * m / (d + 1e-20f)) : (s * m / (1.f - d + 1e-20f));
}

__global__ void gather_cols_kernel(const float* __restrict__ in, int64_t in_rs, float* __restrict__ out,
                                   int64_t out_rs, const int32_t* __restrict__ cols, int ncols,
                                   int64_t rows) {
  const int lane = threadIdx.x & 31;
  const int64_t warp = ((int64_t)blockIdx.x * blockDim.x + threadIdx.x) >> 5;
  const int64_t nwarps = ((int64_t)gridDim.x * blockDim.x) >> 5;
  for (int64_t r = warp; r < rows; r += nwarps)
    for (int j = lane; j < ncols; j += 32) out[r * out_rs + j] = in[r * in_rs + cols[j]];
}

__global__ void scatter_cols_add_kernel(const float* __restrict__ go, int64_t go_rs,
                                        float* __restrict__ gi, int64_t gi_rs,
                                        const int32_t* __restrict__ cols, int ncols, int64_t rows) {
  const int lane = threadIdx.x & 31;
  const int64_t warp = ((int64_t)blockIdx.x * blockDim.x + threadIdx.x) >> 5;
  const int64_t nwarps = ((int64_t)gridDim.x * blockDim.x) >> 5;
  for (int64_t r = warp; r < rows; r += nwarps)
    for (int j = lane; j < ncols; j += 32) gi[r * gi_rs + cols[j]] += go[r * go_rs + j];
}

static inline int grid_for(int64_t work, int threads) {
  int64_t b = (work + threads - 1) / threads;
  if (b < 1) b = 1;
  if (b > RED_MAX_BLOCKS) b = RED_MAX_BLOCKS;
  return (int)b;
}

static inline int bce_blocks(int64_t rows) { return grid_for(rows, RED_THREADS); }
static inline int sse_blocks(int64_t rows, int D) { return grid_for(rows * D, RED_THREADS * 4); }

static int launch_bce(const float* Dv, const float* mask, int64_t M, int halves, int kind0, int kind1, const float* scale,
                      float* gD, RedWs* ws0, RedWs* ws1, cudaStream_t st) {
  const int nbh = bce_blocks(M);
  GANTTS_PDL_LAUNCH((bce_fwd_bwd_kernel), nbh * halves, RED_THREADS, 0, st, Dv, mask, M, kind0, kind1, nbh, scale, gD, ws0, ws1);
  GANTTS_LAUNCH_CHECK("bce_fwd_bwd_kernel");
  return GANTTS_OK;
}

static int launch_sse(const float* a, int64_t a_rs, const float* b, int64_t b_rs, const float* mask, int64_t rows, int D,
                      const float* scale, float* ga, int64_t ga_rs, RedWs* ws, cudaStream_t st,
                      const ColList* bmap = nullptr) {
  ColList none;
  none.n = 0;
  GANTTS_PDL_LAUNCH((sse_fwd_bwd_kernel), sse_blocks(rows, D), RED_THREADS, 0, st, a, a_rs, b, b_rs, mask, rows, D, scale, ga, ga_rs, ws,
                                                                 bmap ? *bmap : none);
  GANTTS_LAUNCH_CHECK("sse_fwd_bwd_kernel");
  return GANTTS_OK;
}

}

using namespace gantts;

extern "C" int gantts_sequence_mask(const int64_t* lengths_dev, float* mask, int B, int T, void* stream) {
  GANTTS_CHECK_ARG(lengths_dev && mask && B >= 1 && T >= 1, "sequence_mask: bad arguments");
  int64_t n = (int64_t)B * T;
  GANTTS_PDL_LAUNCH((sequence_mask_kernel), (unsigned)((n + 255) / 256), 256, 0, as_stream(stream), lengths_dev, mask, B, T);
  GANTTS_LAUNCH_CHECK("sequence_mask_kernel");
  return GANTTS_OK;
}

extern "C" size_t gantts_masked_sse_workspace_bytes(void) { return sizeof(RedWs); }

extern "C" int gantts_masked_sse_fwd(const float* a, int64_t a_rs, const float* b, int64_t b_rs,
                                     const float* mask, int64_t rows, int D, float* sums_dev,
                                     void* workspace, size_t workspace_bytes, void* stream) {
  GANTTS_CHECK_ARG(a && b && mask && sums_dev && rows >= 1 && D >= 1, "masked_sse_fwd: bad arguments");
  if (!workspace || workspace_bytes < sizeof(RedWs)) {
    set_error("masked_sse_fwd: workspace too small (%zu < %zu)", workspace_bytes, sizeof(RedWs));
    return GANTTS_E_WORKSPACE;
  }
  const int nb = sse_blocks(rows, D);
  RedWs* ws = static_cast<RedWs*>(workspace);
  ColList none;
  none.n = 0;
  sse_fwd_bwd_kernel<<<nb, RED_THREADS, 0, as_stream(stream)>>>(a, a_rs, b, b_rs, mask, rows, D, nullptr, nullptr, 0, ws,
                                                                none);
  GANTTS_LAUNCH_CHECK("sse_fwd_bwd_kernel");
  reduce_finish_kernel<<<1, RED_THREADS, 0, as_stream(stream)>>>(ws, nb, sums_dev, 2);
  GANTTS_LAUNCH_CHECK("reduce_finish_kernel");
  return GANTTS_OK;
}

extern "C" int gantts_masked_sse_bwd(const float* a, int64_t a_rs, const float* b, int64_t b_rs,
                                     const float* mask, int64_t rows, int D, const float* scale_dev,
                                     float* grad_a, int64_t ga_rs, int accumulate, void* stream) {
  GANTTS_CHECK_ARG(a && b && mask && scale_dev && grad_a && rows >= 1 && D >= 1,
                   "masked_sse_bwd: bad arguments");
  int nb = grid_for(rows * D, RED_THREADS * 4);
  masked_sse_bwd_kernel<<<nb, RED_THREADS, 0, as_stream(stream)>>>(a, a_rs, b, b_rs, mask, rows, D,
                                                                  scale_dev, grad_a, ga_rs, accumulate);
  GANTTS_LAUNCH_CHECK("masked_sse_bwd_kernel");
  return GANTTS_OK;
}

extern "C" int gantts_masked_bce_fwd(const float* D, const float* mask, int64_t rows, int kind,
                                     float* out_dev, void* workspace, size_t workspace_bytes,
                                     void* stream) {
  GANTTS_CHECK_ARG(D && mask && out_dev && rows >= 1 && (kind == 0 || kind == 1),
                   "masked_bce_fwd: bad arguments");
  if (!workspace || workspace_bytes < sizeof(RedWs)) {
    set_error("masked_bce_fwd: workspace too small");
    return GANTTS_E_WORKSPACE;
  }
  const int nb = bce_blocks(rows);
  RedWs* ws = static_cast<RedWs*>(workspace);
  bce_fwd_bwd_kernel<<<nb, RED_THREADS, 0, as_stream(stream)>>>(D, mask, rows, kind, kind, nb, nullptr, nullptr, ws,
                                                                nullptr);
  GANTTS_LAUNCH_CHECK("bce_fwd_bwd_kernel");
  reduce_finish_kernel<<<1, RED_THREADS, 0, as_stream(stream)>>>(ws, nb, out_dev, 3);
  GANTTS_LAUNCH_CHECK("reduce_finish_kernel");
  return GANTTS_OK;
}

extern "C" int gantts_masked_bce_bwd(const float* D, const float* mask, int64_t rows, int kind,
                                     const float* scale_dev, float* grad_D, void* stream) {
  GANTTS_CHECK_ARG(D && mask && scale_dev && grad_D && rows >= 1 && (kind == 0 || kind == 1),
                   "masked_bce_bwd: bad arguments");
  masked_bce_bwd_kernel<<<(unsigned)((rows + 255) / 256), 256, 0, as_stream(stream)>>>(D, mask, rows, kind,
                                                                                     scale_dev, grad_D);
  GANTTS_LAUNCH_CHECK("masked_bce_bwd_kernel");
  return GANTTS_OK;
}

extern "C" int gantts_gather_cols(const float* in, int64_t in_rs, float* out, int64_t out_rs,
                                  const int32_t* cols_dev, int ncols, int64_t rows, void* stream) {
  GANTTS_CHECK_ARG(in && out && cols_dev && ncols >= 1 && rows >= 1, "gather_cols: bad arguments");
  int nb = grid_for(rows * ncols, 256 * 4);
  gather_cols_kernel<<<nb, 256, 0, as_stream(stream)>>>(in, in_rs, out, out_rs, cols_dev, ncols, rows);
  GANTTS_LAUNCH_CHECK("gather_cols_kernel");
  return GANTTS_OK;
}

extern "C" int gantts_scatter_cols_add(const float* gout, int64_t go_rs, float* gin, int64_t gi_rs,
                                       const int32_t* cols_dev, int ncols, int64_t rows, void* stream) {
  GANTTS_CHECK_ARG(gout && gin && cols_dev && ncols >= 1 && rows >= 1, "scatter_cols_add: bad arguments");
  int nb = grid_for(rows * ncols, 256 * 4);
  scatter_cols_add_kernel<<<nb, 256, 0, as_stream(stream)>>>(gout, go_rs, gin, gi_rs, cols_dev, ncols, rows);
  GANTTS_LAUNCH_CHECK("scatter_cols_add_kernel");
  return GANTTS_OK;
}
```

### gantts_b200/csrc/mlp_tc.cu

```cuda
#include "common.cuh"

namespace gantts {

__global__ void grad_out_to_planes_kernel(const float* __restrict__ gy, int64_t gy_rs,
                                          const float* __restrict__ y, int64_t y_rs, int64_t rows, int cols,
                                          __nv_bfloat16* __restrict__ hi, __nv_bfloat16* __restrict__ lo,
                                          int64_t pitch, int sigmoid) {
  if (cols < 32) {
    const int64_t total = rows * cols;
    for (int64_t i = (int64_t)blockIdx.x * blockDim.x + threadIdx.x; i < total;
         i += (int64_t)gridDim.x * blockDim.x) {
      const int64_t r = i / cols;
      const int c = (int)(i - r * cols);
      float v = gy[r * gy_rs + c];
      if (sigmoid) {
        const float yy = y[r * y_rs + c];
        v *= yy * (1.f - yy);
      }
      const __nv_bfloat16 h = __float2bfloat16_rn(v);
      hi[r * pitch + c] = h;
      lo[r * pitch + c] = __float2bfloat16_rn(v - __bfloat162float(h));
    }
    return;
  }
  const int lane = threadIdx.x & 31;
  const int64_t warp = ((int64_t)blockIdx.x * blockDim.x + threadIdx.x) >> 5;
  const int64_t nwarps = ((int64_t)gridDim.x * blockDim.x) >> 5;
  for (int64_t r = warp; r < rows; r += nwarps)
    for (int c = lane; c < cols; c += 32) {
      float v = gy[r * gy_rs + c];
      if (sigmoid) {
        const float yy = y[r * y_rs + c];
        v *= yy * (1.f - yy);
      }
      const __nv_bfloat16 h = __float2bfloat16_rn(v);
      hi[r * pitch + c] = h;
      lo[r * pitch + c] = __float2bfloat16_rn(v - __bfloat162float(h));
    }
}

__global__ void splitk_reduce_strided_kernel(const float* __restrict__ partial, int nsplit, int stride, int off, int n,
                                             float* __restrict__ out, int accumulate) {
  const int i = blockIdx.x * blockDim.x + threadIdx.x;
  if (i >= n) return;
  float s = 0.f;
  for (int z = 0; z < nsplit; ++z) s += partial[(int64_t)z * stride + off + i];
  out[i] = accumulate ? out[i] + s : s;
}

__global__ void __launch_bounds__(256)
colsum_planes_partial_kernel(const __nv_bfloat16* __restrict__ hi, const __nv_bfloat16* __restrict__ lo,
                             int64_t pitch, int64_t M, int N, int64_t rows_per_chunk,
                             float* __restrict__ partial) {
  __shared__ float sm[8][33];
  const int cx = threadIdx.x & 31, ry = threadIdx.x >> 5;
  const int col = blockIdx.x * 32 + cx;
  const int64_t rbeg = (int64_t)blockIdx.y * rows_per_chunk;
  const int64_t rend = rbeg + rows_per_chunk < M ? rbeg + rows_per_chunk : M;
  float s = 0.f;
  if (col < N)
    for (int64_t r = rbeg + ry; r < rend; r += 8)
      s += __bfloat162float(hi[r * pitch + col]) + __bfloat162float(lo[r * pitch + col]);
  sm[ry][cx] = s;
  __syncthreads();
  if (ry == 0 && col < N) {
    float t = 0.f;
#pragma unroll
    for (int k = 0; k < 8; ++k) t += sm[k][cx];
    partial[(int64_t)blockIdx.y * N + col] = t;
  }
}

struct WeightSplitList {
  int n;
  const float* W[GANTTS_MAX_LAYERS];
  int N[GANTTS_MAX_LAYERS], K[GANTTS_MAX_LAYERS];
  __nv_bfloat16 *hi[GANTTS_MAX_LAYERS], *lo[GANTTS_MAX_LAYERS];
  __nv_bfloat16 *thi[GANTTS_MAX_LAYERS], *tlo[GANTTS_MAX_LAYERS];
  int64_t pitch[GANTTS_MAX_LAYERS], tpitch[GANTTS_MAX_LAYERS];
  int64_t off[GANTTS_MAX_LAYERS + 1];
};

__global__ void __launch_bounds__(256) split_weights_kernel(WeightSplitList wl) {
  pdl_entry();
  __shared__ uint16_t th[32][34], tl[32][34];
  const int cx = threadIdx.x & 31, ry = threadIdx.x >> 5;
  for (int64_t tile = blockIdx.x; tile < wl.off[wl.n]; tile += gridDim.x) {
    int l = 0;
    while (l + 1 < wl.n && tile >= wl.off[l + 1]) ++l;
    const int N = wl.N[l], K = wl.K[l];
    const int tk = (K + 31) / 32;
    const int64_t tt = tile - wl.off[l];
    const int r0 = (int)(tt / tk) * 32, c0 = (int)(tt % tk) * 32;
#pragma unroll
    for (int i = 0; i < 4; ++i) {
      const int r = r0 + ry + 8 * i, c = c0 + cx;
      uint16_t hb = 0, lb = 0;
      if (r < N && c < K) {
        const float v = wl.W[l][(int64_t)r * K + c];
        const __nv_bfloat16 h = __float2bfloat16_rn(v);
        const __nv_bfloat16 lo = __float2bfloat16_rn(v - __bfloat162float(h));
        wl.hi[l][r * wl.pitch[l] + c] = h;
        wl.lo[l][r * wl.pitch[l] + c] = lo;
        hb = __bfloat16_as_ushort(h);
        lb = __bfloat16_as_ushort(lo);
      }
      th[ry + 8 * i][cx] = hb;
      tl[ry + 8 * i][cx] = lb;
    }
    __syncthreads();
#pragma unroll
    for (int i = 0; i < 4; ++i) {
      const int c = c0 + ry + 8 * i, r = r0 + cx;
      if (c < K && r < N) {
        wl.thi[l][(int64_t)c * wl.tpitch[l] + r] = __ushort_as_bfloat16(th[cx][ry + 8 * i]);
        wl.tlo[l][(int64_t)c * wl.tpitch[l] + r] = __ushort_as_bfloat16(tl[cx][ry + 8 * i]);
      }
    }
    __syncthreads();
  }
}

constexpr int GEMV_THREADS = 256;
constexpr int GEMV_MAX_K = 1024;

__global__ void __launch_bounds__(GEMV_THREADS)
gemv_fwd_kernel(const __nv_bfloat16* __restrict__ hi, const __nv_bfloat16* __restrict__ lo, int64_t pitch,
                const float* __restrict__ w, const float* __restrict__ b, float* __restrict__ y, int64_t y_rs,
                int64_t M, int K, int sigmoid) {
  __shared__ float ws[GEMV_MAX_K];
  for (int i = threadIdx.x; i < K; i += GEMV_THREADS) ws[i] = w[i];
  __syncthreads();
  const int lane = threadIdx.x & 31;
  const int64_t warp = ((int64_t)blockIdx.x * GEMV_THREADS + threadIdx.x) >> 5;
  const int64_t nwarps = ((int64_t)gridDim.x * GEMV_THREADS) >> 5;
  const float bias = b[0];
  for (int64_t r = warp; r < M; r += nwarps) {
    const uint32_t* hr = reinterpret_cast<const uint32_t*>(hi + r * pitch);
    const uint32_t* lr = reinterpret_cast<const uint32_t*>(lo + r * pitch);
    float acc = 0.f;
    for (int c = 2 * lane; c < K; c += 64) {
      const uint32_t h2 = hr[c >> 1], l2 = lr[c >> 1];
      const float a0 = __uint_as_float(h2 << 16) + __uint_as_float(l2 << 16);
      const float a1 = __uint_as_float(h2 & 0xffff0000u) + __uint_as_float(l2 & 0xffff0000u);
      acc = fmaf(a0, ws[c], acc);
      if (c + 1 < K) acc = fmaf(a1, ws[c + 1], acc);
    }
    acc = warp_sum(acc);
    if (lane == 0) {
      float z = acc + bias;
      y[r * y_rs] = sigmoid ? 1.f / (1.f + expf(-z)) : z;
    }
  }
}

__global__ void __launch_bounds__(GEMV_THREADS)
gemv_bwd_kernel(const float* __restrict__ gy, int64_t gy_rs, const float* __restrict__ y, int64_t y_rs,
                const __nv_bfloat16* __restrict__ hi, const __nv_bfloat16* __restrict__ lo, int64_t pitch,
                const uint32_t* __restrict__ code, int64_t code_pitch, const float* __restrict__ w,
                __nv_bfloat16* __restrict__ ghi, __nv_bfloat16* __restrict__ glo, int64_t gpitch,
                float* __restrict__ partial, int64_t M, int K, int sigmoid, float dpos, float dneg, float dzero,
                int want_gw) {
  __shared__ float ws[GEMV_MAX_K];
  __shared__ float gws[GEMV_THREADS / 32][GEMV_MAX_K + 1];
  for (int i = threadIdx.x; i < K; i += GEMV_THREADS) ws[i] = w[i];
  const int lane = threadIdx.x & 31, wid = threadIdx.x >> 5;
  for (int i = lane; i <= K; i += 32) gws[wid][i] = 0.f;
  __syncthreads();
  const int64_t warp = ((int64_t)blockIdx.x * GEMV_THREADS + threadIdx.x) >> 5;
  const int64_t nwarps = ((int64_t)gridDim.x * GEMV_THREADS) >> 5;
  float gsum = 0.f;
  for (int64_t r = warp; r < M; r += nwarps) {
    float g = gy[r * gy_rs];
    if (sigmoid) {
      const float yy = y[r * y_rs];
      g *= yy * (1.f - yy);
    }
    gsum += g;
    const uint32_t* hr = reinterpret_cast<const uint32_t*>(hi + r * pitch);
    const uint32_t* lr = reinterpret_cast<const uint32_t*>(lo + r * pitch);
    uint32_t* gh = reinterpret_cast<uint32_t*>(ghi + r * gpitch);
    uint32_t* gl = reinterpret_cast<uint32_t*>(glo + r * gpitch);
    for (int c = 2 * lane; c < K; c += 64) {
      if (want_gw) {
        const uint32_t h2 = hr[c >> 1], l2 = lr[c >> 1];
        const float a0 = __uint_as_float(h2 << 16) + __uint_as_float(l2 << 16);
        const float a1 = __uint_as_float(h2 & 0xffff0000u) + __uint_as_float(l2 & 0xffff0000u);
        gws[wid][c] = fmaf(g, a0, gws[wid][c]);
        if (c + 1 < K) gws[wid][c + 1] = fmaf(g, a1, gws[wid][c + 1]);
      }
      const uint32_t cw = code[r * code_pitch + (c >> 4)];
      const uint32_t c0 = (cw >> (2 * (c & 15))) & 3u, c1 = (cw >> (2 * ((c + 1) & 15))) & 3u;
      const float v0 = g * ws[c] * ((c0 & 1u) ? dzero : ((c0 & 2u) ? dneg : dpos));
      const float v1 = (c + 1 < K) ? g * ws[c + 1] * ((c1 & 1u) ? dzero : ((c1 & 2u) ? dneg : dpos)) : 0.f;
      const uint32_t hp = pack_bf16x2(v0, v1);
      gh[c >> 1] = hp;
      gl[c >> 1] = pack_bf16x2(v0 - __uint_as_float(hp << 16), v1 - __uint_as_float(hp & 0xffff0000u));
    }
  }
  if (want_gw) {
    if (lane == 0) gws[wid][K] = gsum;
    __syncthreads();
    for (int i = threadIdx.x; i <= K; i += GEMV_THREADS) {
      float s = 0.f;
#pragma unroll
      for (int q = 0; q < GEMV_THREADS / 32; ++q) s += gws[q][i];
      partial[(int64_t)blockIdx.x * (K + 1) + i] = s;
    }
  }
}

__device__ __forceinline__ void unpack8(const uint4& h, const uint4& l, float (&a)[8]) {
  const uint32_t hh[4] = {h.x, h.y, h.z, h.w}, ll[4] = {l.x, l.y, l.z, l.w};
#pragma unroll
  for (int i = 0; i < 4; ++i) {
    a[2 * i] = __uint_as_float(hh[i] << 16) + __uint_as_float(ll[i] << 16);
    a[2 * i + 1] = __uint_as_float(hh[i] & 0xffff0000u) + __uint_as_float(ll[i] & 0xffff0000u);
  }
}

__device__ __forceinline__ uint4 ldg_stream16(const void* p) {
  uint4 v;
  asm volatile("ld.global.nc.L1::no_allocate.v4.u32 {%0,%1,%2,%3}, [%4];"
               : "=r"(v.x), "=r"(v.y), "=r"(v.z), "=r"(v.w)
               : "l"(p));
  return v;
}

template <int NCH, int RU>
__global__ void __launch_bounds__(GEMV_THREADS)
gemv_fwd_vec_kernel(const __nv_bfloat16* __restrict__ hi, const __nv_bfloat16* __restrict__ lo, int64_t pitch,
                    const float* __restrict__ w, const float* __restrict__ b, float* __restrict__ y, int64_t y_rs,
                    int64_t M, int K, int sigmoid) {
  pdl_entry();
  const int lane = threadIdx.x & 31;
  float wr[NCH][8];
#pragma unroll
  for (int ch = 0; ch < NCH; ++ch) {
    const int c = ch * 256 + lane * 8;
#pragma unroll
    for (int j = 0; j < 8; ++j) wr[ch][j] = c < K ? w[c + j] : 0.f;
  }
  const int64_t warp = ((int64_t)blockIdx.x * GEMV_THREADS + threadIdx.x) >> 5;
  const int64_t nwarps = ((int64_t)gridDim.x * GEMV_THREADS) >> 5;
  const float bias = b[0];
  for (int64_t r0 = warp * RU; r0 < M; r0 += nwarps * RU) {
    uint4 h[RU][NCH], l[RU][NCH];
#pragma unroll
    for (int u = 0; u < RU; ++u) {
      const int64_t r = r0 + u < M ? r0 + u : M - 1;
#pragma unroll
      for (int ch = 0; ch < NCH; ++ch) {
        const int c = ch * 256 + lane * 8;
        if (c < K) {
          h[u][ch] = ldg_stream16(hi + r * pitch + c);
          l[u][ch] = ldg_stream16(lo + r * pitch + c);
        } else {
          h[u][ch] = make_uint4(0, 0, 0, 0);
          l[u][ch] = make_uint4(0, 0, 0, 0);
        }
      }
    }
    float acc[RU];
#pragma unroll
    for (int u = 0; u < RU; ++u) {
      acc[u] = 0.f;
#pragma unroll
      for (int ch = 0; ch < NCH; ++ch) {
        float a[8];
        unpack8(h[u][ch], l[u][ch], a);
#pragma unroll
        for (int j = 0; j < 8; ++j) acc[u] = fmaf(a[j], wr[ch][j], acc[u]);
      }
    }
#pragma unroll
    for (int u = 0; u < RU; ++u) acc[u] = warp_sum(acc[u]);
    if (lane == 0) {
#pragma unroll
      for (int u = 0; u < RU; ++u)
        if (r0 + u < M) {
          const float z = acc[u] + bias;
          y[(r0 + u) * y_rs] = sigmoid ? 1.f / (1.f + expf(-z)) : z;
        }
    }
  }
}

template <int NCH, int RU>
__global__ void __launch_bounds__(GEMV_THREADS)
gemv_bwd_vec_kernel(const float* __restrict__ gy, int64_t gy_rs, const float* __restrict__ y, int64_t y_rs,
                    const __nv_bfloat16* __restrict__ hi, const __nv_bfloat16* __restrict__ lo, int64_t pitch,
                    const uint32_t* __restrict__ code, int64_t code_pitch, const float* __restrict__ w,
                    __nv_bfloat16* __restrict__ ghi, __nv_bfloat16* __restrict__ glo, int64_t gpitch,
                    float* __restrict__ partial, int64_t M, int K, int sigmoid, float dpos, float dneg, float dzero,
                    int want_gw) {
  pdl_entry();
  __shared__ float gws[GEMV_THREADS / 32][GEMV_MAX_K + 1];
  const int lane = threadIdx.x & 31, wid = threadIdx.x >> 5;
  float wr[NCH][8], gw[NCH][8];
#pragma unroll
  for (int ch = 0; ch < NCH; ++ch) {
    const int c = ch * 256 + lane * 8;
#pragma unroll
    for (int j = 0; j < 8; ++j) {
      wr[ch][j] = c < K ? w[c + j] : 0.f;
      gw[ch][j] = 0.f;
    }
  }
  const int64_t warp = ((int64_t)blockIdx.x * GEMV_THREADS + threadIdx.x) >> 5;
  const int64_t nwarps = ((int64_t)gridDim.x * GEMV_THREADS) >> 5;
  float gsum = 0.f;
  for (int64_t r0 = warp * RU; r0 < M; r0 += nwarps * RU) {
    uint4 h[RU][NCH], l[RU][NCH];
    uint32_t cw[RU][NCH];
    float g[RU];
#pragma unroll
    for (int u = 0; u < RU; ++u) {
      const bool ok = r0 + u < M;
      const int64_t r = ok ? r0 + u : M - 1;
      float gg = ok ? gy[r * gy_rs] : 0.f;
      if (sigmoid) {
        const float yy = y[r * y_rs];
        gg *= yy * (1.f - yy);
      }
      g[u] = gg;
#pragma unroll
      for (int ch = 0; ch < NCH; ++ch) {
        const int c = ch * 256 + lane * 8;
        if (c < K) {
          if (want_gw) {
            h[u][ch] = ldg_stream16(hi + r * pitch + c);
            l[u][ch] = ldg_stream16(lo + r * pitch + c);
          }
          cw[u][ch] = __ldg(code + r * code_pitch + (c >> 4)) >> (2 * (c & 15));
        }
      }
    }
#pragma unroll
    for (int u = 0; u < RU; ++u) {
      gsum += g[u];
      if (r0 + u >= M) continue;
      const int64_t r = r0 + u;
#pragma unroll
      for (int ch = 0; ch < NCH; ++ch) {
        const int c = ch * 256 + lane * 8;
        if (c >= K) continue;
        if (want_gw) {
          float a[8];
          unpack8(h[u][ch], l[u][ch], a);
#pragma unroll
          for (int j = 0; j < 8; ++j) gw[ch][j] = fmaf(g[u], a[j], gw[ch][j]);
        }
        uint32_t oh[4], ol[4];
#pragma unroll
        for (int j = 0; j < 4; ++j) {
          const uint32_t c0 = (cw[u][ch] >> (4 * j)) & 3u, c1 = (cw[u][ch] >> (4 * j + 2)) & 3u;
          const float v0 = g[u] * wr[ch][2 * j] * ((c0 & 1u) ? dzero : ((c0 & 2u) ? dneg : dpos));
          const float v1 = g[u] * wr[ch][2 * j + 1] * ((c1 & 1u) ? dzero : ((c1 & 2u) ? dneg : dpos));
          oh[j] = pack_bf16x2(v0, v1);
          ol[j] = pack_bf16x2(v0 - __uint_as_float(oh[j] << 16), v1 - __uint_as_float(oh[j] & 0xffff0000u));
        }
        *reinterpret_cast<uint4*>(ghi + r * gpitch + c) = make_uint4(oh[0], oh[1], oh[2], oh[3]);
        *reinterpret_cast<uint4*>(glo + r * gpitch + c) = make_uint4(ol[0], ol[1], ol[2], ol[3]);
      }
    }
  }
  if (want_gw) {
#pragma unroll
    for (int ch = 0; ch < NCH; ++ch) {
      const int c = ch * 256 + lane * 8;
      if (c < K) {
#pragma unroll
        for (int j = 0; j < 8; ++j) gws[wid][c + j] = gw[ch][j];
      }
    }
    if (lane == 0) gws[wid][K] = gsum;
    __syncthreads();
    for (int i = threadIdx.x; i <= K; i += GEMV_THREADS) {
      float s = 0.f;
#pragma unroll
      for (int q = 0; q < GEMV_THREADS / 32; ++q) s += gws[q][i];
      partial[(int64_t)blockIdx.x * (K + 1) + i] = s;
    }
  }
}

__global__ void __launch_bounds__(256)
gemv_partial_reduce_kernel(const float* __restrict__ partial, int blocks, int K, float* __restrict__ out_w,
                           float* __restrict__ out_b, int accumulate) {
  pdl_entry();
  __shared__ float sm[8][33];
  const int cl = threadIdx.x & 31, rg = threadIdx.x >> 5;
  const int c = blockIdx.x * 32 + cl;
  float s = 0.f;
  if (c <= K)
    for (int b = rg; b < blocks; b += 8) s += partial[(int64_t)b * (K + 1) + c];
  sm[rg][cl] = s;
  __syncthreads();
  if (rg == 0 && c <= K) {
    float t = 0.f;
#pragma unroll
    for (int q = 0; q < 8; ++q) t += sm[q][cl];
    float* o = c < K ? (out_w ? out_w + c : nullptr) : out_b;
    if (o) *o = accumulate ? *o + t : t;
  }
}

constexpr int GEMV_BLOCKS = 132 * 2;

constexpr int MLP_COLSUM_CHUNKS = 128;
constexpr int MLP_GRAD_BUFS = 2;

static int colsum_planes(const Planes& G, float* gb, int accumulate, float* partial, cudaStream_t st) {
  int chunks = MLP_COLSUM_CHUNKS;
  int64_t rpc = (G.rows + chunks - 1) / chunks;
  if (rpc < 8) rpc = 8;
  chunks = (int)((G.rows + rpc - 1) / rpc);
  dim3 grid((unsigned)((G.cols + 31) / 32), chunks);
  colsum_planes_partial_kernel<<<grid, 256, 0, st>>>(G.hi, G.lo, G.pitch, G.rows, (int)G.cols, rpc, partial);
  GANTTS_LAUNCH_CHECK("colsum_planes_partial_kernel");
  splitk_reduce_kernel<<<(unsigned)((G.cols + 1023) / 1024), 256, 0, st>>>(partial, chunks, G.cols, gb, accumulate);
  GANTTS_LAUNCH_CHECK("splitk_reduce_kernel(colsum planes)");
  return GANTTS_OK;
}

struct MlpTape {
  uint32_t* code[GANTTS_MAX_LAYERS];
  int64_t code_pitch[GANTTS_MAX_LAYERS];
  Planes H[GANTTS_MAX_LAYERS];
  Planes W[GANTTS_MAX_LAYERS];
  Planes Wt[GANTTS_MAX_LAYERS];
};

static int check_mlp(const gantts_mlp_t* m, int64_t M) {
  GANTTS_CHECK_ARG(m, "mlp: null descriptor");
  GANTTS_CHECK_ARG(m->num_layers >= 1 && m->num_layers <= GANTTS_MAX_LAYERS, "mlp: bad layer count %d", m->num_layers);
  GANTTS_CHECK_ARG(M >= 1, "mlp: M must be >= 1");
  for (int l = 0; l <= m->num_layers; ++l) GANTTS_CHECK_ARG(m->dims[l] >= 1, "mlp: bad dim[%d]", l);
  for (int l = 0; l < m->num_layers; ++l) {
    GANTTS_CHECK_ARG(m->W[l] && m->b[l], "mlp: null weight/bias of layer %d", l);
    GANTTS_CHECK_ARG((reinterpret_cast<uintptr_t>(m->b[l]) & 15) == 0, "mlp: bias %d must be 16-byte aligned", l);
  }
  GANTTS_CHECK_ARG(m->dropout_p >= 0.f && m->dropout_p < 1.f, "mlp: dropout p out of [0,1)");
  GANTTS_CHECK_ARG(m->last_act == GANTTS_ACT_NONE || m->last_act == GANTTS_ACT_SIGMOID, "mlp: bad last_act");
  return GANTTS_OK;
}

static size_t carve_tape(const gantts_mlp_t* m, int64_t M, char* base, MlpTape* t) {
  char* cur = base;
  for (int l = 0; l < m->num_layers; ++l) {
    Planes p = carve_planes(cur, M, m->dims[l]);
    if (t) t->H[l] = p;
    const int64_t cp = ((m->dims[l] + 15) / 16 + 3) / 4 * 4;
    if (t) {
      t->code[l] = reinterpret_cast<uint32_t*>(cur);
      t->code_pitch[l] = cp;
    }
    if (l >= 1) cur += ((size_t)M * cp * sizeof(uint32_t) + 255) / 256 * 256;
  }
  for (int l = 0; l < m->num_layers; ++l) {
    Planes a = carve_planes(cur, m->dims[l + 1], m->dims[l]);
    Planes b = carve_planes(cur, m->dims[l], m->dims[l + 1]);
    if (t) { t->W[l] = a; t->Wt[l] = b; }
  }
  return (size_t)(cur - base);
}

static inline uint64_t layer_seed(uint64_t seed, int l) { return seed + 0x9E3779B97F4A7C15ull * (uint64_t)(l + 1); }

}

using namespace gantts;

extern "C" uint64_t gantts_mlp_layer_seed(uint64_t seed, int layer) { return layer_seed(seed, layer); }

extern "C" size_t gantts_mlp_tape_bytes(const gantts_mlp_t* m, int64_t M) {
  if (!m || m->num_layers < 1 || m->num_layers > GANTTS_MAX_LAYERS || M < 1) return 0;
  return carve_tape(m, M, nullptr, nullptr) + 512;
}

namespace gantts {
static size_t mlp_workspace_bytes(const gantts_mlp_t* m, int64_t M, bool upto) {
  if (!m || m->num_layers < 1 || m->num_layers > GANTTS_MAX_LAYERS || M < 1) return 0;
  int maxd = 0;
  size_t part = 0;
  for (int l = 0; l <= m->num_layers; ++l) maxd = m->dims[l] > maxd ? m->dims[l] : maxd;
  for (int l = 0; l < m->num_layers; ++l)
    part += (upto ? mn_partial_bytes_upto(M, m->dims[l + 1], m->dims[l])
                  : mn_partial_bytes(M, m->dims[l + 1], m->dims[l], nullptr, nullptr)) + 256;
  return (size_t)2 * MLP_GRAD_BUFS * plane_bytes(M, maxd) + part + (size_t)MLP_COLSUM_CHUNKS * maxd * sizeof(float) +
         (size_t)GEMV_BLOCKS * (GEMV_MAX_K + 1) * sizeof(float) + 4096;
}
}

extern "C" size_t gantts_mlp_workspace_bytes(const gantts_mlp_t* m, int64_t M) { return mlp_workspace_bytes(m, M, false); }

namespace gantts {
static int mlp_fwd_impl(const gantts_mlp_t* m, const float* x, int64_t x_rs, int64_t M, float* y, int64_t y_rs, void* tape,
                        size_t tape_bytes, void* stream, bool input_ready);

static int mlp_tape_input_planes(const gantts_mlp_t* m, int64_t M, void* tape, size_t tape_bytes, Planes* out) {
  int rc = check_mlp(m, M);
  if (rc) return rc;
  if (!tape || tape_bytes < gantts_mlp_tape_bytes(m, M)) {
    set_error("mlp_tape_input_planes: tape too small");
    return GANTTS_E_WORKSPACE;
  }
  MlpTape t;
  carve_tape(m, M, reinterpret_cast<char*>((reinterpret_cast<uintptr_t>(tape) + 255) / 256 * 256), &t);
  *out = t.H[0];
  return GANTTS_OK;
}
}

extern "C" int gantts_mlp_fwd(const gantts_mlp_t* m, const float* x, int64_t x_rs, int64_t M, float* y,
                              int64_t y_rs, void* tape, size_t tape_bytes, void* stream) {
  GANTTS_CHECK_ARG(m && x && x_rs >= m->dims[0], "mlp_fwd: bad input pointer/stride");
  return mlp_fwd_impl(m, x, x_rs, M, y, y_rs, tape, tape_bytes, stream, false);
}

static int gantts::mlp_fwd_impl(const gantts_mlp_t* m, const float* x, int64_t x_rs, int64_t M, float* y, int64_t y_rs,
                                void* tape, size_t tape_bytes, void* stream, bool input_ready) {
  int rc = check_mlp(m, M);
  if (rc) return rc;
  GANTTS_CHECK_ARG((x || input_ready) && y && y_rs >= m->dims[m->num_layers], "mlp_fwd: bad pointers/strides");
  size_t need = gantts_mlp_tape_bytes(m, M);
  if (!tape || tape_bytes < need) {
    set_error("mlp_fwd: tape too small (%zu < %zu)", tape_bytes, need);
    return GANTTS_E_WORKSPACE;
  }
  cudaStream_t st = as_stream(stream);
  MlpTape t;
  carve_tape(m, M, reinterpret_cast<char*>((reinterpret_cast<uintptr_t>(tape) + 255) / 256 * 256), &t);
  const int L = m->num_layers;
  if (!input_ready && (rc = launch_split(x, x_rs, M, m->dims[0], t.H[0], 0, st))) return rc;
  {
    WeightSplitList wl;
    wl.n = L;
    wl.off[0] = 0;
    for (int l = 0; l < L; ++l) {
      wl.W[l] = m->W[l];
      wl.N[l] = m->dims[l + 1];
      wl.K[l] = m->dims[l];
      wl.hi[l] = t.W[l].hi;
      wl.lo[l] = t.W[l].lo;
      wl.pitch[l] = t.W[l].pitch;
      wl.thi[l] = t.Wt[l].hi;
      wl.tlo[l] = t.Wt[l].lo;
      wl.tpitch[l] = t.Wt[l].pitch;
      wl.off[l + 1] = wl.off[l] + (int64_t)((m->dims[l + 1] + 31) / 32) * ((m->dims[l] + 31) / 32);
    }
    int nb = (int)wl.off[L];
    if (nb > num_sms() * 8) nb = num_sms() * 8;
    if (nb < 1) nb = 1;
    GANTTS_PDL_LAUNCH((split_weights_kernel), nb, 256, 0, st, wl);
    GANTTS_LAUNCH_CHECK("split_weights_kernel");
  }
  for (int l = 0; l < L; ++l) {
    EpiArgs e;
    e.bias = m->b[l];
    if (l < L - 1) {
      e.epi = EPI_PLANES_FWD;
      e.out_hi = t.H[l + 1].hi;
      e.out_lo = t.H[l + 1].lo;
      e.out_pitch = t.H[l + 1].pitch;
      e.code = t.code[l + 1];
      e.code_pitch = t.code_pitch[l + 1];
      e.act = GANTTS_ACT_LEAKY_DROPOUT;
      e.slope = m->slope;
      e.p = m->dropout_p;
      e.seed = layer_seed(m->seed, l);
    } else {
      if (m->dims[L] == 1 && L >= 2 && m->dims[l] <= GEMV_MAX_K && (m->dims[l] & 1) == 0) {
        const int Kl = m->dims[l], sg = m->last_act == GANTTS_ACT_SIGMOID;
        if (Kl % 8 == 0 && Kl <= 256)
          GANTTS_PDL_LAUNCH((gemv_fwd_vec_kernel<1, 4>), 2 * GEMV_BLOCKS, GEMV_THREADS, 0, st, t.H[l].hi, t.H[l].lo, t.H[l].pitch, m->W[l],
                                                                          m->b[l], y, y_rs, M, Kl, sg);
        else if (Kl % 8 == 0 && Kl <= 512)
          gemv_fwd_vec_kernel<2, 2><<<2 * GEMV_BLOCKS, GEMV_THREADS, 0, st>>>(t.H[l].hi, t.H[l].lo, t.H[l].pitch, m->W[l],
                                                                          m->b[l], y, y_rs, M, Kl, sg);
        else if (Kl % 8 == 0)
          gemv_fwd_vec_kernel<4, 1><<<2 * GEMV_BLOCKS, GEMV_THREADS, 0, st>>>(t.H[l].hi, t.H[l].lo, t.H[l].pitch, m->W[l],
                                                                          m->b[l], y, y_rs, M, Kl, sg);
        else
          gemv_fwd_kernel<<<GEMV_BLOCKS, GEMV_THREADS, 0, st>>>(t.H[l].hi, t.H[l].lo, t.H[l].pitch, m->W[l], m->b[l], y,
                                                                y_rs, M, Kl, sg);
        GANTTS_LAUNCH_CHECK("gemv_fwd_kernel");
        continue;
      }
      e.epi = EPI_F32;
      e.C = y;
      e.ldc = y_rs;
      e.act = m->last_act;
    }
    if ((rc = launch_gemm_kk(t.H[l], t.W[l], e, st))) return rc;
  }
  return GANTTS_OK;
}

namespace gantts {
static int mlp_bwd_impl(const gantts_mlp_t* m, const float* gy, int64_t gy_rs, const float* y, int64_t y_rs, int64_t M,
                        const void* tape, size_t tape_bytes, float* gx, int64_t gx_rs, int64_t gx_row0,
                        float* const* gW, float* const* gb, int accumulate, void* workspace, size_t workspace_bytes,
                        void* stream, int gx_accumulate = -1, bool gy_planes_ready = false);
static int mlp_bwd_gy_planes(const gantts_mlp_t* m, int64_t M, void* workspace, size_t workspace_bytes, Planes* out);
}

static int gantts::mlp_bwd_gy_planes(const gantts_mlp_t* m, int64_t M, void* workspace, size_t workspace_bytes, Planes* out) {
  int rc = check_mlp(m, M);
  if (rc) return rc;
  if (!workspace || workspace_bytes < gantts_mlp_workspace_bytes(m, M)) {
    set_error("mlp_bwd_gy_planes: workspace too small");
    return GANTTS_E_WORKSPACE;
  }
  char* cur = reinterpret_cast<char*>((reinterpret_cast<uintptr_t>(workspace) + 255) / 256 * 256);
  *out = carve_planes(cur, M, m->dims[m->num_layers]);
  return GANTTS_OK;
}

extern "C" int gantts_mlp_bwd(const gantts_mlp_t* m, const float* gy, int64_t gy_rs, const float* y,
                              int64_t y_rs, int64_t M, const void* tape, size_t tape_bytes, float* gx,
                              int64_t gx_rs, float* const* gW, float* const* gb, int accumulate,
                              void* workspace, size_t workspace_bytes, void* stream) {
  return mlp_bwd_impl(m, gy, gy_rs, y, y_rs, M, tape, tape_bytes, gx, gx_rs, 0, gW, gb, accumulate, workspace,
                      workspace_bytes, stream, -1);
}

static int gantts::mlp_bwd_impl(const gantts_mlp_t* m, const float* gy, int64_t gy_rs, const float* y, int64_t y_rs,
                                int64_t M, const void* tape, size_t tape_bytes, float* gx, int64_t gx_rs,
                                int64_t gx_row0, float* const* gW, float* const* gb, int accumulate, void* workspace,
                                size_t workspace_bytes, void* stream, int gx_accumulate, bool gy_planes_ready) {
  if (gx_accumulate < 0) gx_accumulate = accumulate;
  int rc = check_mlp(m, M);
  GANTTS_CHECK_ARG(gx_row0 >= 0 && gx_row0 < M, "mlp_bwd: bad gx_row0");
  if (rc) return rc;
  const int L = m->num_layers;
  GANTTS_CHECK_ARG(gy_planes_ready || (gy && gy_rs >= m->dims[L]), "mlp_bwd: bad gy");
  GANTTS_CHECK_ARG(!gy_planes_ready || (m->last_act == GANTTS_ACT_NONE && m->dims[L] > 1),
                   "mlp_bwd: gy planes are only accepted for a linear multi-column output");
  GANTTS_CHECK_ARG(m->last_act != GANTTS_ACT_SIGMOID || y, "mlp_bwd: sigmoid output needs y");
  if (!tape || tape_bytes < gantts_mlp_tape_bytes(m, M)) {
    set_error("mlp_bwd: tape too small");
    return GANTTS_E_WORKSPACE;
  }
  size_t need = gantts_mlp_workspace_bytes(m, M);
  if (!workspace || workspace_bytes < need) {
    set_error("mlp_bwd: workspace too small (%zu < %zu)", workspace_bytes, need);
    return GANTTS_E_WORKSPACE;
  }
  cudaStream_t st = as_stream(stream);
  MlpTape t;
  carve_tape(m, M, reinterpret_cast<char*>((reinterpret_cast<uintptr_t>(const_cast<void*>(tape)) + 255) / 256 * 256), &t);
  int maxd = 0;
  for (int l = 0; l <= L; ++l) maxd = m->dims[l] > maxd ? m->dims[l] : maxd;
  char* cur = reinterpret_cast<char*>((reinterpret_cast<uintptr_t>(workspace) + 255) / 256 * 256);
  char* gbuf[MLP_GRAD_BUFS];
  for (int i = 0; i < MLP_GRAD_BUFS; ++i) {
    gbuf[i] = cur;
    cur += 2 * plane_bytes(M, maxd);
  }
  float* colpart = reinterpret_cast<float*>(cur);
  cur += ((size_t)MLP_COLSUM_CHUNKS * maxd * sizeof(float) + 255) / 256 * 256;
  char* partial_cur = cur;
  ReduceList rl;

  float* gemv_part = reinterpret_cast<float*>(partial_cur);
  partial_cur += ((size_t)GEMV_BLOCKS * (GEMV_MAX_K + 1) * sizeof(float) + 255) / 256 * 256;
  int pp = 0;
  int l_start = L - 1;
  char* c0 = gbuf[pp];
  Planes G = carve_planes(c0, M, m->dims[L]);
  if (m->dims[L] == 1 && L >= 2 && m->dims[L - 1] <= GEMV_MAX_K && (m->dims[L - 1] & 1) == 0) {
    const int K1 = m->dims[L - 1];
    char* cg = gbuf[pp];
    G = carve_planes(cg, M, K1);
    const float ks = m->dropout_p > 0.f ? 1.f / (1.f - m->dropout_p) : 1.f;
    const int want = (gW && gW[L - 1]) || (gb && gb[L - 1]);
#define GANTTS_GEMV_BWD_ARGS                                                                                     \
  gy, gy_rs, y, y_rs, t.H[L - 1].hi, t.H[L - 1].lo, t.H[L - 1].pitch, t.code[L - 1], t.code_pitch[L - 1],       \
      m->W[L - 1], G.hi, G.lo, G.pitch, gemv_part, M, K1, m->last_act == GANTTS_ACT_SIGMOID ? 1 : 0, ks,        \
      m->slope * ks, m->dropout_p > 0.f ? 0.f : m->slope, want
    if (K1 % 8 == 0 && K1 <= 256)
      GANTTS_PDL_LAUNCH((gemv_bwd_vec_kernel<1, 4>), GEMV_BLOCKS, GEMV_THREADS, 0, st, GANTTS_GEMV_BWD_ARGS);
    else if (K1 % 8 == 0 && K1 <= 512)
      gemv_bwd_vec_kernel<2, 2><<<GEMV_BLOCKS, GEMV_THREADS, 0, st>>>(GANTTS_GEMV_BWD_ARGS);
    else if (K1 % 8 == 0)
      gemv_bwd_vec_kernel<4, 1><<<GEMV_BLOCKS, GEMV_THREADS, 0, st>>>(GANTTS_GEMV_BWD_ARGS);
    else
      gemv_bwd_kernel<<<GEMV_BLOCKS, GEMV_THREADS, 0, st>>>(GANTTS_GEMV_BWD_ARGS);
#undef GANTTS_GEMV_BWD_ARGS
    GANTTS_LAUNCH_CHECK("gemv_bwd_kernel");
    if (want) {
      GANTTS_PDL_LAUNCH((gemv_partial_reduce_kernel), (K1 + 1 + 31) / 32, 256, 0, st, gemv_part, GEMV_BLOCKS, K1,
                                                                    gW ? gW[L - 1] : nullptr,
                                                                    gb ? gb[L - 1] : nullptr, accumulate);
      GANTTS_LAUNCH_CHECK("gemv_partial_reduce_kernel");
    }
    l_start = L - 2;
  } else if (!gy_planes_ready) {
    int64_t total = M * m->dims[L];
    int nb = (int)((total + 1023) / 1024);
    if (nb > num_sms() * 8) nb = num_sms() * 8;
    if (nb < 1) nb = 1;
    grad_out_to_planes_kernel<<<nb, 256, 0, st>>>(gy, gy_rs, y, y_rs, M, m->dims[L], G.hi, G.lo, G.pitch,
                                                  m->last_act == GANTTS_ACT_SIGMOID ? 1 : 0);
    GANTTS_LAUNCH_CHECK("grad_out_to_planes_kernel");
  }
  for (int l = l_start; l >= 0; --l) {
    float* gbl = (gb && gb[l]) ? gb[l] : nullptr;
    if (gW && gW[l]) {
      float* partial = reinterpret_cast<float*>(partial_cur);
      partial_cur += mn_partial_bytes(M, m->dims[l + 1], m->dims[l], nullptr, nullptr) + 256;
      if ((rc = launch_gemm_mn(G, t.H[l], gW[l], gbl, accumulate, partial, st, &rl))) return rc;
    } else if (gbl) {
      if ((rc = colsum_planes(G, gbl, accumulate, colpart, st))) return rc;
    }
    if (l > 0) {
      char* c1 = gbuf[pp ^ 1];
      Planes Gn = carve_planes(c1, M, m->dims[l]);
      EpiArgs e;
      e.epi = EPI_PLANES_BWD;
      e.out_hi = Gn.hi;
      e.out_lo = Gn.lo;
      e.out_pitch = Gn.pitch;
      e.code = t.code[l];
      e.code_pitch = t.code_pitch[l];
      e.slope = m->slope;
      e.p = m->dropout_p;
      if ((rc = launch_gemm_kk(G, t.Wt[l], e, st))) return rc;
      G = Gn;
      pp ^= 1;
    } else if (gx) {
      EpiArgs e;
      e.epi = EPI_F32;
      e.C = gx + gx_row0 * gx_rs;
      e.ldc = gx_rs;
      e.accumulate = gx_accumulate;
      Planes Gs = G;
      Gs.hi += gx_row0 * G.pitch;
      Gs.lo += gx_row0 * G.pitch;
      Gs.rows = G.rows - gx_row0;
      if ((rc = launch_gemm_kk(Gs, t.Wt[0], e, st))) return rc;
    }
  }
  return flush_reduce(rl, accumulate, st);
}
```

Measured before the change: 15.86 million.

## Fuse discriminator GEMV head, sigmoid, BCE loss and head backward into one kernel

For a non-RNN discriminator whose last layer is a single sigmoid unit, one d_head_kernel now computes the output GEMV, sigmoid, BCE loss partials, the gradient of the loss and the head-layer backward (input-gradient planes and weight-gradient partials). The MLP forward stops before the head and the backward skips the separate gemv_bwd kernel. This removes the separate GEMV forward, BCE and GEMV backward launches, along with the round trips of d_out and g_dout through global memory. In exchange it adds a large templated kernel with heavy register use, and the finalize step now uses GEMV_BLOCKS partial counts.

```diff
diff --git a/gantts_b200/csrc/gan_step.cu b/gantts_b200/csrc/gan_step.cu
--- a/gantts_b200/csrc/gan_step.cu
+++ b/gantts_b200/csrc/gan_step.cu
@@ -981,6 +981,7 @@
   bool has_d, has_adv;
   bool train;
   bool adv_window;
+  bool d_head;
   HighwayArgs hwa;
   ColList static_cols, adv_cols, real_cols;
   uint64_t seed;
@@ -1004,8 +1005,9 @@
 static int step_finalize(const Step& s, float* losses_dev) {
   const gantts_gan_step_t* c = s.c;
   RedCounts cnt{};
-  if (s.has_d) cnt.n[R_REAL] = cnt.n[R_FAKE] = bce_blocks(s.M);
-  if (s.has_adv) cnt.n[R_ADV] = bce_blocks(s.M);
+  const int bce_parts = s.d_head ? GEMV_BLOCKS : bce_blocks(s.M);
+  if (s.has_d) cnt.n[R_REAL] = cnt.n[R_FAKE] = bce_parts;
+  if (s.has_adv) cnt.n[R_ADV] = bce_parts;
   cnt.n[R_MGE] = sse_blocks(s.M, s.nS);
   cnt.n[R_MSE] = sse_blocks(s.M, s.d_out);
   GANTTS_PDL_LAUNCH((finalize_losses_kernel), 1, RED_THREADS, 0, s.st, s.L.scal, losses_dev, s.L.red, cnt,
@@ -1105,7 +1107,7 @@
       GANTTS_LAUNCH_CHECK("gather_planes_kernel(adv)");
     }
     if (s.d_rnn() && (rc = discriminator_stack_fwd(s, stacked, nullptr, tape_in))) return rc;
-    return mlp_fwd_impl(&s.d, nullptr, 0, rows, L.d_out, 1, L.d_tape, L.d_tape_bytes, s.stream, true);
+    return mlp_fwd_impl(&s.d, nullptr, 0, rows, L.d_out, 1, L.d_tape, L.d_tape_bytes, s.stream, true, s.d_head);
   }
   const int dD = s.dD;
   if (stacked) {
@@ -1122,7 +1124,23 @@
     if ((rc = discriminator_stack_fwd(s, stacked, L.d_in + (stacked ? 0 : M * dD), tape_in))) return rc;
     return mlp_fwd_impl(&s.d, nullptr, 0, rows, L.d_out, 1, L.d_tape, L.d_tape_bytes, s.stream, true);
   }
-  return gantts_mlp_fwd(&s.d, L.d_in + (stacked ? 0 : M * dD), dD, rows, L.d_out, 1, L.d_tape, L.d_tape_bytes, s.stream);
+  return mlp_fwd_impl(&s.d, L.d_in + (stacked ? 0 : M * dD), dD, rows, L.d_out, 1, L.d_tape, L.d_tape_bytes, s.stream, false,
+                      s.d_head);
+}
+
+static int discriminator_loss(Step& s, bool stacked, bool eval = false) {
+  const StepLayout& L = s.L;
+  const int64_t M = s.M;
+  const float* scale = eval ? nullptr : L.scal + (stacked ? S_INV_T : S_ADV_SCALE);
+  RedWs* ws0 = &L.red[stacked ? R_REAL : R_ADV];
+  RedWs* ws1 = stacked ? &L.red[R_FAKE] : nullptr;
+  RedWs* ws_adv = eval && s.has_adv ? &L.red[R_ADV] : nullptr;
+  if (s.d_head)
+    return mlp_d_head(&s.d, stacked ? 2 * M : M, L.d_out, L.d_tape, L.d_tape_bytes,
+                      DHeadLoss{L.mask, M, 0, 1, scale, ws0, ws1, ws_adv}, stacked && !eval, L.mlp_ws, L.mlp_ws_bytes, s.st);
+  int rc = launch_bce(L.d_out, L.mask, M, stacked ? 2 : 1, 0, 1, scale, eval ? nullptr : L.g_dout, ws0, ws1, s.st);
+  if (rc || !ws_adv) return rc;
+  return launch_bce(L.d_out + M, L.mask, M, 1, 0, 0, nullptr, nullptr, ws_adv, nullptr, s.st);
 }
 
 static int discriminator_bwd(Step& s, bool stacked, bool input_grad = true) {
@@ -1147,7 +1165,7 @@
                              input_grad ? &din : nullptr, s.st)))
       return rc;
   } else if ((rc = mlp_bwd_impl(&s.d, L.g_dout, 1, L.d_out, 1, skip + M, L.d_tape, L.d_tape_bytes, gx, s.adv_window ? s.nS : s.dD,
-                                skip, gW, gb, 0, L.mlp_ws, L.mlp_ws_bytes, s.stream, s.adv_window ? 1 : -1))) {
+                                skip, gW, gb, 0, L.mlp_ws, L.mlp_ws_bytes, s.stream, s.adv_window ? 1 : -1, false, s.d_head))) {
     return rc;
   }
   if (s.adv_window || !input_grad) return GANTTS_OK;
@@ -1274,6 +1292,8 @@
     GANTTS_CHECK_ARG(s.adv_cols.c[i] >= 0 && s.adv_cols.c[i] < c->n_static_cols, "gan_step: adversarial column out of range");
     s.real_cols.c[i] = s.static_cols.c[s.adv_cols.c[i]];
   }
+  const char* dh = getenv("GANTTS_B200_D_HEAD");
+  s.d_head = s.has_d && !s.d_rnn() && gemv_head(&c->d) && !(dh && atoi(dh) == 0);
   s.g.seed = gantts_gan_step_seed(seed, 0);
   const cudaStream_t st = s.st;
 
@@ -1286,11 +1306,7 @@
     if ((rc = generator_fwd(s, false))) return rc;
     if (s.has_d) {
       if ((rc = discriminator_fwd(s, true))) return rc;
-      if ((rc = launch_bce(L.d_out, L.mask, M, 2, 0, 1, L.scal + S_INV_T, nullptr, &L.red[R_REAL], &L.red[R_FAKE], st)))
-        return rc;
-      if (s.has_adv &&
-          (rc = launch_bce(L.d_out + M, L.mask, M, 1, 0, 0, L.scal + S_INV_T, nullptr, &L.red[R_ADV], nullptr, st)))
-        return rc;
+      if ((rc = discriminator_loss(s, true, true))) return rc;
     }
     if ((rc = launch_sse(y_hat_static, nS, y, s.d_out, L.mask, M, nS, L.scal + S_MGE_SCALE, nullptr, 0, &L.red[R_MGE], st,
                          &s.static_cols)))
@@ -1314,8 +1330,7 @@
     if (s.has_d) {
       s.d.seed = gantts_gan_step_seed(seed, 1);
       if ((rc = discriminator_fwd(s, true))) return rc;
-      if ((rc = launch_bce(L.d_out, L.mask, M, 2, 0, 1, L.scal + S_INV_T, L.g_dout, &L.red[R_REAL], &L.red[R_FAKE], st)))
-        return rc;
+      if ((rc = discriminator_loss(s, true))) return rc;
       if ((rc = discriminator_bwd(s, true, !d_only))) return rc;
     }
   }
@@ -1337,8 +1352,7 @@
     if (s.has_adv) {
       s.d.seed = gantts_gan_step_seed(seed, 2);
       if ((rc = discriminator_fwd(s, false))) return rc;
-      if ((rc = launch_bce(L.d_out, L.mask, M, 1, 0, 0, L.scal + S_ADV_SCALE, L.g_dout, &L.red[R_ADV], nullptr, st)))
-        return rc;
+      if ((rc = discriminator_loss(s, false))) return rc;
       if ((rc = discriminator_bwd(s, false))) return rc;
     }
     if ((rc = generator_bwd(s))) return rc;
diff --git a/gantts_b200/csrc/losses.cu b/gantts_b200/csrc/losses.cu
--- a/gantts_b200/csrc/losses.cu
+++ b/gantts_b200/csrc/losses.cu
@@ -93,6 +93,15 @@
   }
 }
 
+__device__ __forceinline__ float bce_term(float dv, float m, int kind, float s, float (&v)[RED_NV]) {
+  const float arg = kind == 0 ? (dv + 1e-20f) : (1.f - dv + 1e-20f);
+  v[0] -= logf(arg) * m;
+  const bool hit = kind == 0 ? (dv > 0.5f) : (dv < 0.5f);
+  v[1] += hit ? m : 0.f;
+  v[2] += m;
+  return kind == 0 ? (-s * m / (dv + 1e-20f)) : (s * m / (1.f - dv + 1e-20f));
+}
+
 __global__ void __launch_bounds__(RED_THREADS)
 bce_fwd_bwd_kernel(const float* __restrict__ Dv, const float* __restrict__ mask, int64_t M, int kind0, int kind1,
                    int nbh, const float* __restrict__ scale, float* __restrict__ gD, RedWs* ws0, RedWs* ws1) {
@@ -106,13 +115,8 @@
   const float s = g ? scale[0] : 0.f;
   float v[RED_NV] = {0.f, 0.f, 0.f, 0.f};
   for (int64_t i = (int64_t)blk * RED_THREADS + threadIdx.x; i < M; i += (int64_t)nbh * RED_THREADS) {
-    const float dv = d[i], m = mask[i];
-    const float arg = kind == 0 ? (dv + 1e-20f) : (1.f - dv + 1e-20f);
-    v[0] -= logf(arg) * m;
-    const bool hit = kind == 0 ? (dv > 0.5f) : (dv < 0.5f);
-    v[1] += hit ? m : 0.f;
-    v[2] += m;
-    if (g) g[i] = kind == 0 ? (-s * m / (dv + 1e-20f)) : (s * m / (1.f - dv + 1e-20f));
+    const float gv = bce_term(d[i], mask[i], kind, s, v);
+    if (g) g[i] = gv;
   }
   block_sum<RED_NV>(v, sm);
   if (threadIdx.x == 0) {
@@ -127,8 +131,8 @@
                                       float* __restrict__ gD) {
   int64_t i = (int64_t)blockIdx.x * blockDim.x + threadIdx.x;
   if (i >= rows) return;
-  float d = Dv[i], m = mask[i], s = scale[0];
-  gD[i] = kind == 0 ? (-s * m / (d + 1e-20f)) : (s * m / (1.f - d + 1e-20f));
+  float v[RED_NV] = {0.f, 0.f, 0.f, 0.f};
+  gD[i] = bce_term(Dv[i], mask[i], kind, scale[0], v);
 }
 
 __global__ void gather_cols_kernel(const float* __restrict__ in, int64_t in_rs, float* __restrict__ out,
diff --git a/gantts_b200/csrc/mlp_tc.cu b/gantts_b200/csrc/mlp_tc.cu
--- a/gantts_b200/csrc/mlp_tc.cu
+++ b/gantts_b200/csrc/mlp_tc.cu
@@ -408,6 +408,214 @@
 
 constexpr int GEMV_BLOCKS = 132 * 2;
 
+struct DHeadArgs {
+  const __nv_bfloat16 *hi, *lo;
+  int64_t pitch;
+  const uint32_t* code;
+  int64_t code_pitch;
+  const float *w, *b;
+  float* d_out;
+  const float* mask;
+  int64_t M, rows;
+  int K;
+  int kind0, kind1;
+  const float* scale;
+  RedWs *ws0, *ws1;
+  RedWs* ws_adv;
+  __nv_bfloat16 *ghi, *glo;
+  int64_t gpitch;
+  float* partial;
+  float dpos, dneg, dzero;
+};
+
+template <int CW>
+__device__ __forceinline__ void load_planes(const __nv_bfloat16* hi, const __nv_bfloat16* lo, uint32_t (&h)[CW / 2],
+                                            uint32_t (&l)[CW / 2]) {
+  if constexpr (CW == 8) {
+    const uint4 a = ldg_stream16(hi), b = ldg_stream16(lo);
+    h[0] = a.x, h[1] = a.y, h[2] = a.z, h[3] = a.w;
+    l[0] = b.x, l[1] = b.y, l[2] = b.z, l[3] = b.w;
+  } else {
+    h[0] = *reinterpret_cast<const uint32_t*>(hi);
+    l[0] = *reinterpret_cast<const uint32_t*>(lo);
+  }
+}
+
+template <int CW>
+__device__ __forceinline__ void unpack_words(const uint32_t (&h)[CW / 2], const uint32_t (&l)[CW / 2], float (&a)[CW]) {
+#pragma unroll
+  for (int i = 0; i < CW / 2; ++i) {
+    a[2 * i] = __uint_as_float(h[i] << 16) + __uint_as_float(l[i] << 16);
+    a[2 * i + 1] = __uint_as_float(h[i] & 0xffff0000u) + __uint_as_float(l[i] & 0xffff0000u);
+  }
+}
+
+template <int CW, int NCH, int RU>
+__device__ __forceinline__ void load_group(const DHeadArgs& a, int64_t r0, int lane, bool bwd, uint32_t (&h)[RU][NCH][CW / 2],
+                                           uint32_t (&l)[RU][NCH][CW / 2], uint32_t (&cw)[RU][NCH], float (&m)[RU]) {
+#pragma unroll
+  for (int u = 0; u < RU; ++u) {
+    const int64_t r = r0 + u < a.rows ? r0 + u : a.rows - 1;
+    m[u] = __ldg(a.mask + (r >= a.M ? r - a.M : r));
+#pragma unroll
+    for (int ch = 0; ch < NCH; ++ch) {
+      const int c = ch * 32 * CW + lane * CW;
+      if (c < a.K) {
+        load_planes<CW>(a.hi + r * a.pitch + c, a.lo + r * a.pitch + c, h[u][ch], l[u][ch]);
+        cw[u][ch] = bwd ? __ldg(a.code + r * a.code_pitch + (c >> 4)) >> (2 * (c & 15)) : 0u;
+      } else {
+#pragma unroll
+        for (int i = 0; i < CW / 2; ++i) h[u][ch][i] = l[u][ch][i] = 0u;
+        cw[u][ch] = 0u;
+      }
+    }
+  }
+}
+
+template <int CW, int NCH, int RU, bool PF = CW * NCH == 8>
+__global__ void __launch_bounds__(GEMV_THREADS, PF ? 2 : 1) d_head_kernel(DHeadArgs a) {
+  pdl_entry();
+  __shared__ float gws[GEMV_THREADS / 32][GEMV_MAX_K + 1];
+  __shared__ float sm[3 * RED_NV * 32];
+  constexpr int CS = 32 * CW;
+  const int lane = threadIdx.x & 31, wid = threadIdx.x >> 5;
+  const int K = a.K;
+  const bool bwd = a.scale != nullptr, want_gw = a.partial != nullptr;
+  float wr[NCH][CW], gw[NCH][CW];
+#pragma unroll
+  for (int ch = 0; ch < NCH; ++ch) {
+    const int c = ch * CS + lane * CW;
+#pragma unroll
+    for (int j = 0; j < CW; ++j) {
+      wr[ch][j] = c < K ? a.w[c + j] : 0.f;
+      gw[ch][j] = 0.f;
+    }
+  }
+  const int64_t warp = ((int64_t)blockIdx.x * GEMV_THREADS + threadIdx.x) >> 5;
+  const int64_t nwarps = ((int64_t)gridDim.x * GEMV_THREADS) >> 5;
+  const float bias = a.b[0];
+  const float s = bwd ? a.scale[0] : 0.f;
+  float v0[RED_NV] = {0.f, 0.f, 0.f, 0.f}, v1[RED_NV] = {0.f, 0.f, 0.f, 0.f}, va[RED_NV] = {0.f, 0.f, 0.f, 0.f};
+  float gsum = 0.f;
+  uint32_t h[RU][NCH][CW / 2], l[RU][NCH][CW / 2], cw[RU][NCH];
+  float mk[RU];
+  if (warp * RU < a.rows) load_group<CW, NCH, RU>(a, warp * RU, lane, bwd, h, l, cw, mk);
+  for (int64_t r0 = warp * RU; r0 < a.rows; r0 += nwarps * RU) {
+    const int64_t rn = r0 + nwarps * RU;
+    uint32_t hn[RU][NCH][CW / 2], ln[RU][NCH][CW / 2], cwn[RU][NCH];
+    float mn[RU];
+    if (PF && rn < a.rows) load_group<CW, NCH, RU>(a, rn, lane, bwd, hn, ln, cwn, mn);
+    float acc[RU];
+#pragma unroll
+    for (int u = 0; u < RU; ++u) {
+      acc[u] = 0.f;
+#pragma unroll
+      for (int ch = 0; ch < NCH; ++ch) {
+        float x[CW];
+        unpack_words<CW>(h[u][ch], l[u][ch], x);
+#pragma unroll
+        for (int j = 0; j < CW; ++j) acc[u] = fmaf(x[j], wr[ch][j], acc[u]);
+      }
+    }
+#pragma unroll
+    for (int u = 0; u < RU; ++u) acc[u] = warp_sum(acc[u]);
+#pragma unroll
+    for (int u = 0; u < RU; ++u) {
+      float g = 0.f;
+      if (r0 + u < a.rows) {
+        const int64_t r = r0 + u;
+        const bool fake = r >= a.M;
+        const float z = acc[u] + bias;
+        const float dv = 1.f / (1.f + expf(-z));
+        if (lane == 0) a.d_out[r] = dv;
+        const float m = mk[u];
+        const float gd = fake ? bce_term(dv, m, a.kind1, s, v1) : bce_term(dv, m, a.kind0, s, v0);
+        if (fake && a.ws_adv) bce_term(dv, m, 0, 0.f, va);
+        if (bwd) g = gd * (dv * (1.f - dv));
+      }
+      gsum += g;
+      if (!bwd || r0 + u >= a.rows) continue;
+      const int64_t r = r0 + u;
+#pragma unroll
+      for (int ch = 0; ch < NCH; ++ch) {
+        const int c = ch * CS + lane * CW;
+        if (c >= K) continue;
+        if (want_gw) {
+          float x[CW];
+          unpack_words<CW>(h[u][ch], l[u][ch], x);
+#pragma unroll
+          for (int j = 0; j < CW; ++j) gw[ch][j] = fmaf(g, x[j], gw[ch][j]);
+        }
+        uint32_t oh[CW / 2], ol[CW / 2];
+#pragma unroll
+        for (int j = 0; j < CW / 2; ++j) {
+          const uint32_t c0 = (cw[u][ch] >> (4 * j)) & 3u, c1 = (cw[u][ch] >> (4 * j + 2)) & 3u;
+          const float p0 = g * wr[ch][2 * j] * ((c0 & 1u) ? a.dzero : ((c0 & 2u) ? a.dneg : a.dpos));
+          const float p1 = g * wr[ch][2 * j + 1] * ((c1 & 1u) ? a.dzero : ((c1 & 2u) ? a.dneg : a.dpos));
+          oh[j] = pack_bf16x2(p0, p1);
+          ol[j] = pack_bf16x2(p0 - __uint_as_float(oh[j] << 16), p1 - __uint_as_float(oh[j] & 0xffff0000u));
+        }
+        if constexpr (CW == 8) {
+          *reinterpret_cast<uint4*>(a.ghi + r * a.gpitch + c) = make_uint4(oh[0], oh[1], oh[2], oh[3]);
+          *reinterpret_cast<uint4*>(a.glo + r * a.gpitch + c) = make_uint4(ol[0], ol[1], ol[2], ol[3]);
+        } else {
+          *reinterpret_cast<uint32_t*>(a.ghi + r * a.gpitch + c) = oh[0];
+          *reinterpret_cast<uint32_t*>(a.glo + r * a.gpitch + c) = ol[0];
+        }
+      }
+    }
+    if (!PF && rn < a.rows) {
+      load_group<CW, NCH, RU>(a, rn, lane, bwd, h, l, cw, mk);
+    } else if (rn < a.rows) {
+#pragma unroll
+      for (int u = 0; u < RU; ++u) {
+        mk[u] = mn[u];
+#pragma unroll
+        for (int ch = 0; ch < NCH; ++ch) {
+          cw[u][ch] = cwn[u][ch];
+#pragma unroll
+          for (int i = 0; i < CW / 2; ++i) h[u][ch][i] = hn[u][ch][i], l[u][ch][i] = ln[u][ch][i];
+        }
+      }
+    }
+  }
+  if (want_gw) {
+#pragma unroll
+    for (int ch = 0; ch < NCH; ++ch) {
+      const int c = ch * CS + lane * CW;
+      if (c < K) {
+#pragma unroll
+        for (int j = 0; j < CW; ++j) gws[wid][c + j] = gw[ch][j];
+      }
+    }
+    if (lane == 0) gws[wid][K] = gsum;
+    __syncthreads();
+    for (int i = threadIdx.x; i <= K; i += GEMV_THREADS) {
+      float t = 0.f;
+#pragma unroll
+      for (int q = 0; q < GEMV_THREADS / 32; ++q) t += gws[q][i];
+      a.partial[(int64_t)blockIdx.x * (K + 1) + i] = t;
+    }
+  }
+  float v[3 * RED_NV];
+#pragma unroll
+  for (int k = 0; k < RED_NV; ++k) {
+    v[k] = lane == 0 ? v0[k] : 0.f;
+    v[RED_NV + k] = lane == 0 ? v1[k] : 0.f;
+    v[2 * RED_NV + k] = lane == 0 ? va[k] : 0.f;
+  }
+  block_sum<3 * RED_NV>(v, sm);
+  if (threadIdx.x == 0) {
+    RedWs* const ws[3] = {a.ws0, a.rows > a.M ? a.ws1 : nullptr, a.ws_adv};
+#pragma unroll
+    for (int q = 0; q < 3; ++q)
+      if (ws[q]) {
+#pragma unroll
+        for (int k = 0; k < RED_NV; ++k) ws[q]->partial[blockIdx.x][k] = v[q * RED_NV + k];
+      }
+  }
+}
+
 constexpr int MLP_COLSUM_CHUNKS = 128;
 constexpr int MLP_GRAD_BUFS = 2;
 
@@ -468,6 +676,35 @@
 
 static inline uint64_t layer_seed(uint64_t seed, int l) { return seed + 0x9E3779B97F4A7C15ull * (uint64_t)(l + 1); }
 
+static inline bool gemv_head(const gantts_mlp_t* m) {
+  const int L = m->num_layers, K = m->dims[L - 1];
+  return m->dims[L] == 1 && L >= 2 && K <= GEMV_MAX_K && (K & 1) == 0;
+}
+
+struct MlpBwdWs {
+  char* gbuf[MLP_GRAD_BUFS];
+  float* colpart;
+  float* gemv_part;
+  char* partial;
+};
+
+static MlpBwdWs carve_bwd_ws(const gantts_mlp_t* m, int64_t M, void* workspace) {
+  int maxd = 0;
+  for (int l = 0; l <= m->num_layers; ++l) maxd = m->dims[l] > maxd ? m->dims[l] : maxd;
+  char* cur = reinterpret_cast<char*>((reinterpret_cast<uintptr_t>(workspace) + 255) / 256 * 256);
+  MlpBwdWs w;
+  for (int i = 0; i < MLP_GRAD_BUFS; ++i) {
+    w.gbuf[i] = cur;
+    cur += 2 * plane_bytes(M, maxd);
+  }
+  w.colpart = reinterpret_cast<float*>(cur);
+  cur += ((size_t)MLP_COLSUM_CHUNKS * maxd * sizeof(float) + 255) / 256 * 256;
+  w.gemv_part = reinterpret_cast<float*>(cur);
+  cur += ((size_t)GEMV_BLOCKS * (GEMV_MAX_K + 1) * sizeof(float) + 255) / 256 * 256;
+  w.partial = cur;
+  return w;
+}
+
 }
 
 using namespace gantts;
@@ -497,7 +734,7 @@
 
 namespace gantts {
 static int mlp_fwd_impl(const gantts_mlp_t* m, const float* x, int64_t x_rs, int64_t M, float* y, int64_t y_rs, void* tape,
-                        size_t tape_bytes, void* stream, bool input_ready);
+                        size_t tape_bytes, void* stream, bool input_ready, bool stop_before_head = false);
 
 static int mlp_tape_input_planes(const gantts_mlp_t* m, int64_t M, void* tape, size_t tape_bytes, Planes* out) {
   int rc = check_mlp(m, M);
@@ -520,10 +757,12 @@
 }
 
 static int gantts::mlp_fwd_impl(const gantts_mlp_t* m, const float* x, int64_t x_rs, int64_t M, float* y, int64_t y_rs,
-                                void* tape, size_t tape_bytes, void* stream, bool input_ready) {
+                                void* tape, size_t tape_bytes, void* stream, bool input_ready, bool stop_before_head) {
   int rc = check_mlp(m, M);
   if (rc) return rc;
-  GANTTS_CHECK_ARG((x || input_ready) && y && y_rs >= m->dims[m->num_layers], "mlp_fwd: bad pointers/strides");
+  GANTTS_CHECK_ARG(!stop_before_head || gemv_head(m), "mlp_fwd: only a GEMV output unit can be left to the caller");
+  GANTTS_CHECK_ARG((x || input_ready) && (stop_before_head || (y && y_rs >= m->dims[m->num_layers])),
+                   "mlp_fwd: bad pointers/strides");
   size_t need = gantts_mlp_tape_bytes(m, M);
   if (!tape || tape_bytes < need) {
     set_error("mlp_fwd: tape too small (%zu < %zu)", tape_bytes, need);
@@ -556,7 +795,7 @@
     GANTTS_PDL_LAUNCH((split_weights_kernel), nb, 256, 0, st, wl);
     GANTTS_LAUNCH_CHECK("split_weights_kernel");
   }
-  for (int l = 0; l < L; ++l) {
+  for (int l = 0; l < (stop_before_head ? L - 1 : L); ++l) {
     EpiArgs e;
     e.bias = m->b[l];
     if (l < L - 1) {
@@ -571,7 +810,7 @@
       e.p = m->dropout_p;
       e.seed = layer_seed(m->seed, l);
     } else {
-      if (m->dims[L] == 1 && L >= 2 && m->dims[l] <= GEMV_MAX_K && (m->dims[l] & 1) == 0) {
+      if (gemv_head(m)) {
         const int Kl = m->dims[l], sg = m->last_act == GANTTS_ACT_SIGMOID;
         if (Kl % 8 == 0 && Kl <= 256)
           GANTTS_PDL_LAUNCH((gemv_fwd_vec_kernel<1, 4>), 2 * GEMV_BLOCKS, GEMV_THREADS, 0, st, t.H[l].hi, t.H[l].lo, t.H[l].pitch, m->W[l],
@@ -602,7 +841,7 @@
 static int mlp_bwd_impl(const gantts_mlp_t* m, const float* gy, int64_t gy_rs, const float* y, int64_t y_rs, int64_t M,
                         const void* tape, size_t tape_bytes, float* gx, int64_t gx_rs, int64_t gx_row0,
                         float* const* gW, float* const* gb, int accumulate, void* workspace, size_t workspace_bytes,
-                        void* stream, int gx_accumulate = -1, bool gy_planes_ready = false);
+                        void* stream, int gx_accumulate = -1, bool gy_planes_ready = false, bool head_ready = false);
 static int mlp_bwd_gy_planes(const gantts_mlp_t* m, int64_t M, void* workspace, size_t workspace_bytes, Planes* out);
 }
 
@@ -629,16 +868,18 @@
 static int gantts::mlp_bwd_impl(const gantts_mlp_t* m, const float* gy, int64_t gy_rs, const float* y, int64_t y_rs,
                                 int64_t M, const void* tape, size_t tape_bytes, float* gx, int64_t gx_rs,
                                 int64_t gx_row0, float* const* gW, float* const* gb, int accumulate, void* workspace,
-                                size_t workspace_bytes, void* stream, int gx_accumulate, bool gy_planes_ready) {
+                                size_t workspace_bytes, void* stream, int gx_accumulate, bool gy_planes_ready,
+                                bool head_ready) {
   if (gx_accumulate < 0) gx_accumulate = accumulate;
   int rc = check_mlp(m, M);
   GANTTS_CHECK_ARG(gx_row0 >= 0 && gx_row0 < M, "mlp_bwd: bad gx_row0");
   if (rc) return rc;
   const int L = m->num_layers;
-  GANTTS_CHECK_ARG(gy_planes_ready || (gy && gy_rs >= m->dims[L]), "mlp_bwd: bad gy");
+  GANTTS_CHECK_ARG(!head_ready || gemv_head(m), "mlp_bwd: only a GEMV output unit's backward can be ready");
+  GANTTS_CHECK_ARG(gy_planes_ready || head_ready || (gy && gy_rs >= m->dims[L]), "mlp_bwd: bad gy");
   GANTTS_CHECK_ARG(!gy_planes_ready || (m->last_act == GANTTS_ACT_NONE && m->dims[L] > 1),
                    "mlp_bwd: gy planes are only accepted for a linear multi-column output");
-  GANTTS_CHECK_ARG(m->last_act != GANTTS_ACT_SIGMOID || y, "mlp_bwd: sigmoid output needs y");
+  GANTTS_CHECK_ARG(m->last_act != GANTTS_ACT_SIGMOID || y || head_ready, "mlp_bwd: sigmoid output needs y");
   if (!tape || tape_bytes < gantts_mlp_tape_bytes(m, M)) {
     set_error("mlp_bwd: tape too small");
     return GANTTS_E_WORKSPACE;
@@ -651,26 +892,18 @@
   cudaStream_t st = as_stream(stream);
   MlpTape t;
   carve_tape(m, M, reinterpret_cast<char*>((reinterpret_cast<uintptr_t>(const_cast<void*>(tape)) + 255) / 256 * 256), &t);
-  int maxd = 0;
-  for (int l = 0; l <= L; ++l) maxd = m->dims[l] > maxd ? m->dims[l] : maxd;
-  char* cur = reinterpret_cast<char*>((reinterpret_cast<uintptr_t>(workspace) + 255) / 256 * 256);
-  char* gbuf[MLP_GRAD_BUFS];
-  for (int i = 0; i < MLP_GRAD_BUFS; ++i) {
-    gbuf[i] = cur;
-    cur += 2 * plane_bytes(M, maxd);
-  }
-  float* colpart = reinterpret_cast<float*>(cur);
-  cur += ((size_t)MLP_COLSUM_CHUNKS * maxd * sizeof(float) + 255) / 256 * 256;
-  char* partial_cur = cur;
+  const MlpBwdWs w = carve_bwd_ws(m, M, workspace);
+  char* const* gbuf = w.gbuf;
+  float* colpart = w.colpart;
+  float* gemv_part = w.gemv_part;
+  char* partial_cur = w.partial;
   ReduceList rl;
 
-  float* gemv_part = reinterpret_cast<float*>(partial_cur);
-  partial_cur += ((size_t)GEMV_BLOCKS * (GEMV_MAX_K + 1) * sizeof(float) + 255) / 256 * 256;
   int pp = 0;
   int l_start = L - 1;
   char* c0 = gbuf[pp];
   Planes G = carve_planes(c0, M, m->dims[L]);
-  if (m->dims[L] == 1 && L >= 2 && m->dims[L - 1] <= GEMV_MAX_K && (m->dims[L - 1] & 1) == 0) {
+  if (gemv_head(m)) {
     const int K1 = m->dims[L - 1];
     char* cg = gbuf[pp];
     G = carve_planes(cg, M, K1);
@@ -680,16 +913,18 @@
   gy, gy_rs, y, y_rs, t.H[L - 1].hi, t.H[L - 1].lo, t.H[L - 1].pitch, t.code[L - 1], t.code_pitch[L - 1],       \
       m->W[L - 1], G.hi, G.lo, G.pitch, gemv_part, M, K1, m->last_act == GANTTS_ACT_SIGMOID ? 1 : 0, ks,        \
       m->slope * ks, m->dropout_p > 0.f ? 0.f : m->slope, want
-    if (K1 % 8 == 0 && K1 <= 256)
-      GANTTS_PDL_LAUNCH((gemv_bwd_vec_kernel<1, 4>), GEMV_BLOCKS, GEMV_THREADS, 0, st, GANTTS_GEMV_BWD_ARGS);
-    else if (K1 % 8 == 0 && K1 <= 512)
-      gemv_bwd_vec_kernel<2, 2><<<GEMV_BLOCKS, GEMV_THREADS, 0, st>>>(GANTTS_GEMV_BWD_ARGS);
-    else if (K1 % 8 == 0)
-      gemv_bwd_vec_kernel<4, 1><<<GEMV_BLOCKS, GEMV_THREADS, 0, st>>>(GANTTS_GEMV_BWD_ARGS);
-    else
-      gemv_bwd_kernel<<<GEMV_BLOCKS, GEMV_THREADS, 0, st>>>(GANTTS_GEMV_BWD_ARGS);
+    if (!head_ready) {
+      if (K1 % 8 == 0 && K1 <= 256)
+        GANTTS_PDL_LAUNCH((gemv_bwd_vec_kernel<1, 4>), GEMV_BLOCKS, GEMV_THREADS, 0, st, GANTTS_GEMV_BWD_ARGS);
+      else if (K1 % 8 == 0 && K1 <= 512)
+        gemv_bwd_vec_kernel<2, 2><<<GEMV_BLOCKS, GEMV_THREADS, 0, st>>>(GANTTS_GEMV_BWD_ARGS);
+      else if (K1 % 8 == 0)
+        gemv_bwd_vec_kernel<4, 1><<<GEMV_BLOCKS, GEMV_THREADS, 0, st>>>(GANTTS_GEMV_BWD_ARGS);
+      else
+        gemv_bwd_kernel<<<GEMV_BLOCKS, GEMV_THREADS, 0, st>>>(GANTTS_GEMV_BWD_ARGS);
+      GANTTS_LAUNCH_CHECK("gemv_bwd_kernel");
+    }
 #undef GANTTS_GEMV_BWD_ARGS
-    GANTTS_LAUNCH_CHECK("gemv_bwd_kernel");
     if (want) {
       GANTTS_PDL_LAUNCH((gemv_partial_reduce_kernel), (K1 + 1 + 31) / 32, 256, 0, st, gemv_part, GEMV_BLOCKS, K1,
                                                                     gW ? gW[L - 1] : nullptr,
@@ -745,3 +980,77 @@
   }
   return flush_reduce(rl, accumulate, st);
 }
+
+namespace gantts {
+struct DHeadLoss {
+  const float* mask;
+  int64_t M;
+  int kind0, kind1;
+  const float* scale;
+  RedWs *ws0, *ws1;
+  RedWs* ws_adv;
+};
+
+static int mlp_d_head(const gantts_mlp_t* m, int64_t rows, float* y, const void* tape, size_t tape_bytes,
+                      const DHeadLoss& loss, bool want_gw, void* workspace, size_t workspace_bytes, cudaStream_t st) {
+  int rc = check_mlp(m, rows);
+  if (rc) return rc;
+  GANTTS_CHECK_ARG(gemv_head(m) && m->last_act == GANTTS_ACT_SIGMOID, "mlp_d_head: needs a single sigmoid GEMV output unit");
+  GANTTS_CHECK_ARG(y && loss.mask && loss.ws0 && (rows == loss.M || (rows == 2 * loss.M && loss.ws1)) &&
+                       (!loss.ws_adv || rows == 2 * loss.M) && (!want_gw || loss.scale),
+                   "mlp_d_head: bad arguments");
+  if (!tape || tape_bytes < gantts_mlp_tape_bytes(m, rows)) {
+    set_error("mlp_d_head: tape too small");
+    return GANTTS_E_WORKSPACE;
+  }
+  if (loss.scale && (!workspace || workspace_bytes < gantts_mlp_workspace_bytes(m, rows))) {
+    set_error("mlp_d_head: workspace too small");
+    return GANTTS_E_WORKSPACE;
+  }
+  MlpTape t;
+  carve_tape(m, rows, reinterpret_cast<char*>((reinterpret_cast<uintptr_t>(const_cast<void*>(tape)) + 255) / 256 * 256), &t);
+  const int L = m->num_layers, K = m->dims[L - 1];
+  DHeadArgs a{};
+  a.hi = t.H[L - 1].hi;
+  a.lo = t.H[L - 1].lo;
+  a.pitch = t.H[L - 1].pitch;
+  a.code = t.code[L - 1];
+  a.code_pitch = t.code_pitch[L - 1];
+  a.w = m->W[L - 1];
+  a.b = m->b[L - 1];
+  a.d_out = y;
+  a.mask = loss.mask;
+  a.M = loss.M;
+  a.rows = rows;
+  a.K = K;
+  a.kind0 = loss.kind0;
+  a.kind1 = loss.kind1;
+  a.scale = loss.scale;
+  a.ws0 = loss.ws0;
+  a.ws1 = loss.ws1;
+  a.ws_adv = loss.ws_adv;
+  if (loss.scale) {
+    const MlpBwdWs w = carve_bwd_ws(m, rows, workspace);
+    char* cg = w.gbuf[0];
+    const Planes G = carve_planes(cg, rows, K);
+    a.ghi = G.hi;
+    a.glo = G.lo;
+    a.gpitch = G.pitch;
+    a.partial = want_gw ? w.gemv_part : nullptr;
+    const float ks = m->dropout_p > 0.f ? 1.f / (1.f - m->dropout_p) : 1.f;
+    a.dpos = ks;
+    a.dneg = m->slope * ks;
+    a.dzero = m->dropout_p > 0.f ? 0.f : m->slope;
+  }
+  if (K % 8 == 0 && K <= 256)
+    GANTTS_PDL_LAUNCH((d_head_kernel<8, 1, 4>), GEMV_BLOCKS, GEMV_THREADS, 0, st, a);
+  else if (K % 8 == 0 && K <= 512)
+    GANTTS_PDL_LAUNCH((d_head_kernel<8, 2, 2>), GEMV_BLOCKS, GEMV_THREADS, 0, st, a);
+  else if (K % 8 == 0)
+    GANTTS_PDL_LAUNCH((d_head_kernel<8, 4, 1>), GEMV_BLOCKS, GEMV_THREADS, 0, st, a);
+  else
+    GANTTS_PDL_LAUNCH((d_head_kernel<2, GEMV_MAX_K / 64, 1>), GEMV_BLOCKS, GEMV_THREADS, 0, st, a);
+  GANTTS_LAUNCH_CHECK("d_head_kernel");
+  return GANTTS_OK;
+}
+}
```

New measurement: 15.94 million, median of 6. Within noise of the previous version (+0.5%).
